# FurkanOM/tf-ssd

Measured on AMD Instinct MI355X. Metric: images/sec SSD300 (MobileNetV2) fwd+NMS, higher is better.
Workload: dtype f32

## Files before the change

include/ssd_hip.h:

```cpp
#ifndef SSD_HIP_H
#define SSD_HIP_H

#include <stddef.h>
#include <stdint.h>

#ifdef __cplusplus
extern "C" {
#endif

#define SSD_OK 0
#define SSD_E_INVALID (-1)
#define SSD_E_HIP (-2)
#define SSD_E_UNSUPPORTED (-3)
#define SSD_E_STATE (-4)

const char* ssd_version(void);
const char* ssd_last_error(void);
int ssd_init(int device);
void* ssd_stream_create(int high_priority);
void* ssd_stream_create_masked(const unsigned* cu_mask, int words);
int ssd_stream_destroy(void* stream);

int ssd_priors_count(const int* fmaps, const int* n_ars, int levels);
int ssd_priors(const int* fmaps, const float* const* ars, const int* n_ars, int levels,
// ... 364 lines not shown
    int B, H, W, Cin;
    int Cout, kh, kw;
    int stride, dilation;
    int pad_t, pad_l, pad_b, pad_r;
    int act;
    int has_residual;
} ssd_conv_desc;

int ssd_same_pads(int in, int k, int stride, int dilation, int* before, int* after);
int ssd_conv_out_size(int in, int k, int stride, int dilation, int pad_before, int pad_after);

size_t ssd_conv_packed_weight_floats(int kh, int kw, int Cin, int Cout);
int ssd_conv_pack_weights(const float* hwio_dev, int kh, int kw, int Cin, int Cout,
                          float* packed_dev, void* stream);

int ssd_conv2d(const ssd_conv_desc* d, const float* in_dev, const float* packed_w_dev,
               const float* scale_dev, const float* shift_dev, const float* residual_dev,
               float* out_dev, long out_batch_stride, long out_pixel_stride, void* stream);

int ssd_conv_num_configs(void);
const char* ssd_conv_config_name(int config);
int ssd_conv2d_ex(const ssd_conv_desc* d, const float* in_dev, const float* packed_w_dev,
                  const float* scale_dev, const float* shift_dev, const float* residual_dev,
                  float* out_dev, long out_batch_stride, long out_pixel_stride, int config,
                  int split_k, float* splitk_ws_dev, void* stream);

int ssd_split_planes(const float* x_dev, long n, int channels, int planes, void* planes_dev, long plane_stride, void* stream);
int ssd_join_planes(const void* planes_dev, long n, int channels, int planes, long plane_stride, float* x_dev, void* stream);
int ssd_conv2d_planes(const ssd_conv_desc* d, const void* in_planes_dev, int planes, long in_plane_stride,
                      const float* packed_w_dev, const float* scale_dev, const float* shift_dev,
                      const float* residual_dev, float* out_dev, long out_batch_stride, long out_pixel_stride,
                      void* out_planes_dev, long out_plane_stride, int config, int split_k,
                      float* splitk_ws_dev, void* stream);

size_t ssd_conv_f16x2_weight_bytes(int kh, int kw, int Cin, int Cout);
int ssd_conv_pack_weights_f16x2(const float* packed_w_dev, int kh, int kw, int Cin, int Cout, void* w_planes_dev,
                                int* k_out, void* stream);
int ssd_conv2d_planes_f16x2(const ssd_conv_desc* d, const void* in_planes_dev, long in_plane_stride,
                            const float* packed_w_dev, const void* w_planes_dev, int w_exp, const float* scale_dev,
                            const float* shift_dev, const float* residual_dev, float* out_dev,
                            long out_batch_stride, long out_pixel_stride, void* out_planes_dev,
                            long out_plane_stride, int config, int split_k, float* splitk_ws_dev, void* stream);

size_t ssd_conv_wino_weight_floats(int Cin, int Cout);
int ssd_conv_wino_pack_weights(const float* hwio_dev, int Cin, int Cout, float* wino_w_dev, void* stream);
int ssd_conv_wino_num_configs(void);
int ssd_conv2d_wino(const ssd_conv_desc* d, const float* in_dev, const float* wino_w_dev,
                    const float* scale_dev, const float* shift_dev, float* out_dev,
                    long out_batch_stride, long out_pixel_stride, int wino_config, int split_k,
                    float* splitk_ws_dev, void* stream);

int ssd_dwconv3x3(const float* in_dev, int B, int H, int W, int C, int stride,
                  int pad_t, int pad_l, int pad_b, int pad_r,
                  const float* w_dev, const float* scale_dev, const float* shift_dev,
                  int act, float* out_dev, void* stream);

int ssd_maxpool2d(const float* in_dev, int B, int H, int W, int C, int k, int stride,
                  int pad_t, int pad_l, int pad_b, int pad_r, float* out_dev, void* stream);

int ssd_l2norm(const float* in_dev, long pixels, int C, const float* gamma_dev,
               float* out_dev, void* stream);

int ssd_softmax(const float* in_dev, long rows, int L, float* out_dev, void* stream);

typedef struct ssd_net ssd_net;

enum ssd_backbone { SSD_MOBILENET_V2 = 0, SSD_VGG16 = 1 };

ssd_net* ssd_net_create(int backbone, int img_size, int levels, const int* n_ars,
                        int total_labels);
void ssd_net_destroy(ssd_net* net);

int ssd_net_num_params(const ssd_net* net);
const char* ssd_net_param_name(const ssd_net* net, int i);
int ssd_net_param_rank(const ssd_net* net, int i);
const int* ssd_net_param_shape(const ssd_net* net, int i);
int ssd_net_set_param(ssd_net* net, const char* name, const float* host_data, size_t count);
int ssd_net_get_param(const ssd_net* net, const char* name, float* host_out, size_t count);
int ssd_net_finalize(ssd_net* net, int max_batch);
long ssd_net_get_tuning(const ssd_net* net, char* buf, size_t cap);
int ssd_net_set_tuning(ssd_net* net, const char* text);
int ssd_net_tuning_stats(const ssd_net* net, int* from_table, int* timed);
int ssd_net_memory_bytes(const ssd_net* net, size_t out[4]);
const char* ssd_build_id(void);
int ssd_net_num_priors(const ssd_net* net);
int ssd_net_feature_map_size(const ssd_net* net, int level);

int ssd_net_forward(ssd_net* net, const float* image_dev, int B, float* deltas_out_dev,
                    float* probs_out_dev, void* stream);

int ssd_net_predict(ssd_net* net, const float* image_dev, int B, const float* priors_dev,
                    const float* var, int max_total, float iou_thr, float score_thr,
                    float* boxes_dev, float* labels_dev, float* scores_dev, int* valid_dev,
                    void* stream);
int ssd_net_predict_cfg(ssd_net* net, const float* image_dev, int B, const float* priors_dev, const float* var,
                        const ssd_nms_config* cfg, float* boxes_dev, float* labels_dev, float* scores_dev,
                        int* valid_dev, void* stream);

long ssd_net_fetch_activation(ssd_net* net, const char* layer, float* host_out, size_t cap);
long ssd_net_fetch_planes(ssd_net* net, const char* layer, float* host_out, size_t cap, int* planes_out);

int ssd_net_num_layers(const ssd_net* net);
const char* ssd_net_layer_name(const ssd_net* net, int i);
const char* ssd_net_layer_kind(const ssd_net* net, int i);
const char* ssd_net_layer_config(const ssd_net* net, int i);
double ssd_net_layer_flops(const ssd_net* net, int i, int B);
double ssd_net_layer_bytes(const ssd_net* net, int i, int B);
double ssd_net_layer_executed_flops(const ssd_net* net, int i, int B);
int ssd_net_set_option(ssd_net* net, const char* name, int value);
int ssd_net_set_timing(ssd_net* net, int enabled);
int ssd_net_read_timing(ssd_net* net, float* ms_sum_out, int* forwards_out);
int ssd_net_profile_layers(ssd_net* net, const float* image_dev, int B, int reps,
                           float* ms_out, void* stream);

int ssd_net_train_begin(ssd_net* net, int batch);
size_t ssd_net_trainable_floats(const ssd_net* net);
long ssd_net_trainable_offset(const ssd_net* net, const char* name);
int ssd_net_train_forward_backward(ssd_net* net, const float* image_dev, int B,
                                   const float* actual_deltas_dev, const float* actual_labels_dev,
                                   float neg_pos_ratio, float loc_loss_alpha, float* grads_flat_dev,
                                   float* loc_loss_dev, float* conf_loss_dev, void* stream);
int ssd_net_train_forward_backward_cfg(ssd_net* net, const float* image_dev, int B,
                                       const float* actual_deltas_dev, const float* actual_labels_dev,
                                       const ssd_loss_config* loss, float* grads_flat_dev,
                                       float* loc_loss_dev, float* conf_loss_dev, void* stream);
int ssd_net_train_set_buckets(ssd_net* net, int n, const long* lo);
int ssd_net_train_wait_bucket(ssd_net* net, int k, void* stream);
int ssd_net_adam_step(ssd_net* net, const float* grads_flat_dev, float lr, float beta1, float beta2,
                      float eps, float grad_scale, void* stream);
long ssd_net_train_steps(const ssd_net* net);
#define SSD_OPT_ADAM 0
#define SSD_OPT_SGD 1
typedef struct ssd_optimizer {
    int kind;
    float beta1, beta2, eps;
    float momentum;
    int nesterov;
    float clipnorm, clipvalue, global_clipnorm;
} ssd_optimizer;
int ssd_net_optimizer_step(ssd_net* net, const float* grads_flat_dev, const ssd_optimizer* opt, float lr,
                           float grad_scale, void* stream);
int ssd_net_optimizer_reset(ssd_net* net);
long ssd_net_optimizer_get_state(ssd_net* net, const char* slot, float* host_out, size_t cap);
int ssd_net_optimizer_set_state(ssd_net* net, const char* slot, const float* host_in, size_t count);
int ssd_net_train_set_steps(ssd_net* net, long steps);
int ssd_net_train_matrix_flops(const ssd_net* net, double* out3);
int ssd_net_regularization_loss(ssd_net* net, float* host_out);
int ssd_net_set_trainable(ssd_net* net, const char* keras_layer, int trainable);
int ssd_net_get_trainable(const ssd_net* net, const char* keras_layer);
#define SSD_PLAN_WGRAD 1
#define SSD_PLAN_WGRAD2 2
#define SSD_PLAN_DGRAD 4
#define SSD_PLAN_RESGRAD 8
#define SSD_PLAN_BN_BATCH 16
#define SSD_PLAN_BN_PARAMS 32
#define SSD_PLAN_SKIP 64
int ssd_net_train_plan(const ssd_net* net, int layer, int* flags);
long ssd_net_train_fetch(ssd_net* net, const char* what, int B, float* host_out, size_t cap);

int ssd_conv_wgrad_num_configs(void);
size_t ssd_conv_wgrad_workspace_floats(const ssd_conv_desc* d, int N);
int ssd_conv2d_wgrad_ex(const ssd_conv_desc* d, const float* x_dev, const float* g_dev, int ldg, int N, int config,
                        float* dW_dev, float* workspace_dev, size_t workspace_floats, void* stream);
int ssd_dwconv3x3_backward(const float* x_dev, const float* g_dev, const float* w_dev, int B, int H, int W, int C, int stride,
                           int pad_t, int pad_l, int accumulate, float* dx_dev, float* dw_dev, float* workspace_dev,
                           size_t workspace_floats, void* stream);

#ifdef __cplusplus
}
#endif
#endif
```

tf-ssd_amd/csrc/ssd_bf16x3.h:

```cpp
#pragma once
#include <hip/hip_runtime.h>

namespace ssd {

typedef float b3_f32x4 __attribute__((ext_vector_type(4)));
typedef short bf16x8 __attribute__((ext_vector_type(8)));

struct B3 {
    bf16x8 h, m, l;
};

__device__ __forceinline__ void split1(float x, short& h, short& m, short& l) {
    const unsigned hb = __float_as_uint(x) & 0xffff0000u;
    const float r1 = x - __uint_as_float(hb);
    const unsigned mb = __float_as_uint(r1) & 0xffff0000u;
    const float r2 = r1 - __uint_as_float(mb);
    h = (short)(hb >> 16);
    m = (short)(mb >> 16);
    l = (short)(__float_as_uint(r2) >> 16);
}
__device__ __forceinline__ void split4(const b3_f32x4 v, uint2& h, uint2& m, uint2& l) {
    unsigned hb[4], mb[4], lb[4];
#pragma unroll
    for (int j = 0; j < 4; ++j) {
        hb[j] = __float_as_uint(v[j]) & 0xffff0000u;
        const float r1 = v[j] - __uint_as_float(hb[j]);
        mb[j] = __float_as_uint(r1) & 0xffff0000u;
        lb[j] = __float_as_uint(r1 - __uint_as_float(mb[j]));
    }
    h = make_uint2(__builtin_amdgcn_perm(hb[1], hb[0], 0x07060302u), __builtin_amdgcn_perm(hb[3], hb[2], 0x07060302u));
    m = make_uint2(__builtin_amdgcn_perm(mb[1], mb[0], 0x07060302u), __builtin_amdgcn_perm(mb[3], mb[2], 0x07060302u));
    l = make_uint2(__builtin_amdgcn_perm(lb[1], lb[0], 0x07060302u), __builtin_amdgcn_perm(lb[3], lb[2], 0x07060302u));
}
__device__ __forceinline__ B3 split3(const b3_f32x4 a, const b3_f32x4 b) {
    B3 r;
#pragma unroll
    for (int j = 0; j < 4; ++j) {
        short h, m, l;
        split1(a[j], h, m, l);
        r.h[j] = h; r.m[j] = m; r.l[j] = l;
        split1(b[j], h, m, l);
        r.h[4 + j] = h; r.m[4 + j] = m; r.l[4 + j] = l;
    }
    return r;
}
__device__ __forceinline__ b3_f32x4 mma6(const B3& w, const B3& x, b3_f32x4 acc) {
    acc = __builtin_amdgcn_mfma_f32_16x16x32_bf16(w.m, x.m, acc, 0, 0, 0);
    acc = __builtin_amdgcn_mfma_f32_16x16x32_bf16(w.h, x.l, acc, 0, 0, 0);
    acc = __builtin_amdgcn_mfma_f32_16x16x32_bf16(w.l, x.h, acc, 0, 0, 0);
    acc = __builtin_amdgcn_mfma_f32_16x16x32_bf16(w.h, x.m, acc, 0, 0, 0);
    acc = __builtin_amdgcn_mfma_f32_16x16x32_bf16(w.m, x.h, acc, 0, 0, 0);
    acc = __builtin_amdgcn_mfma_f32_16x16x32_bf16(w.h, x.h, acc, 0, 0, 0);
    return acc;
}

typedef __bf16 bf16x2_t __attribute__((ext_vector_type(2)));
typedef float b3_f32x2 __attribute__((ext_vector_type(2)));

__device__ __forceinline__ unsigned rne2(float a, float b) {
    const bf16x2_t r = __builtin_convertvector(b3_f32x2{a, b}, bf16x2_t);
    return __builtin_bit_cast(unsigned, r);
}
__device__ __forceinline__ short rne1(float a) { return (short)(rne2(a, 0.f) & 0xffffu); }
__device__ __forceinline__ uint2 rne4(const b3_f32x4 v) { return make_uint2(rne2(v[0], v[1]), rne2(v[2], v[3])); }

typedef _Float16 f16x2_t __attribute__((ext_vector_type(2)));
typedef _Float16 f16x8 __attribute__((ext_vector_type(8)));
constexpr float kF16x2ActScale = 256.f;

__device__ __forceinline__ void split_h2(const float a, const float b, unsigned& h, unsigned& l) {
    const f16x2_t hh = __builtin_convertvector(b3_f32x2{a, b}, f16x2_t);
    const b3_f32x2 back = __builtin_convertvector(hh, b3_f32x2);
    const f16x2_t ll = __builtin_convertvector(b3_f32x2{a - back[0], b - back[1]}, f16x2_t);
    h = __builtin_bit_cast(unsigned, hh);
    l = __builtin_bit_cast(unsigned, ll);
}
__device__ __forceinline__ void split4_h(const b3_f32x4 v, uint2& h, uint2& l) {
    split_h2(v[0] * kF16x2ActScale, v[1] * kF16x2ActScale, h.x, l.x);
    split_h2(v[2] * kF16x2ActScale, v[3] * kF16x2ActScale, h.y, l.y);
}
__device__ __forceinline__ float join_h(const short h, const short l) {
    const float fh = (float)__builtin_bit_cast(_Float16, h), fl = (float)__builtin_bit_cast(_Float16, l);
    return (fh + fl) * (1.f / kF16x2ActScale);
}

template <int NP>
struct BP {
    bf16x8 p[NP];
};
template <int NP>
__device__ __forceinline__ BP<NP> splitN(const b3_f32x4 a, const b3_f32x4 b) {
    BP<NP> r;
    if constexpr (NP == 3) {
        const B3 s = split3(a, b);
        r.p[0] = s.h; r.p[1] = s.m; r.p[2] = s.l;
    } else {
        const uint4 u = make_uint4(rne2(a[0], a[1]), rne2(a[2], a[3]), rne2(b[0], b[1]), rne2(b[2], b[3]));
        r.p[0] = __builtin_bit_cast(bf16x8, u);
    }
    return r;
}
template <int NP>
__device__ __forceinline__ b3_f32x4 mmaN(const BP<NP>& w, const BP<NP>& x, b3_f32x4 acc) {
    if constexpr (NP == 2) {
        const f16x8 wh = __builtin_bit_cast(f16x8, w.p[0]), wl = __builtin_bit_cast(f16x8, w.p[1]);
        const f16x8 xh = __builtin_bit_cast(f16x8, x.p[0]), xl = __builtin_bit_cast(f16x8, x.p[1]);
        acc = __builtin_amdgcn_mfma_f32_16x16x32_f16(wl, xh, acc, 0, 0, 0);
        acc = __builtin_amdgcn_mfma_f32_16x16x32_f16(wh, xl, acc, 0, 0, 0);
        return __builtin_amdgcn_mfma_f32_16x16x32_f16(wh, xh, acc, 0, 0, 0);
    }
    if constexpr (NP == 3) {
        acc = __builtin_amdgcn_mfma_f32_16x16x32_bf16(w.p[1], x.p[1], acc, 0, 0, 0);
        acc = __builtin_amdgcn_mfma_f32_16x16x32_bf16(w.p[0], x.p[2], acc, 0, 0, 0);
        acc = __builtin_amdgcn_mfma_f32_16x16x32_bf16(w.p[2], x.p[0], acc, 0, 0, 0);
        acc = __builtin_amdgcn_mfma_f32_16x16x32_bf16(w.p[0], x.p[1], acc, 0, 0, 0);
        acc = __builtin_amdgcn_mfma_f32_16x16x32_bf16(w.p[1], x.p[0], acc, 0, 0, 0);
    }
    return __builtin_amdgcn_mfma_f32_16x16x32_bf16(w.p[0], x.p[0], acc, 0, 0, 0);
}
__device__ __forceinline__ void pack_planes(float x, int bf16_mode, short& h, short& m, short& l) {
    if (bf16_mode) { h = rne1(x); m = 0; l = 0; }
    else split1(x, h, m, l);
}

__device__ __host__ __forceinline__ long plane_elem(const long pix, const int c, const long P) {
    return (((long)(c >> 5) * P + pix) << 5) + (c & 31);
}
__device__ __forceinline__ void store_planes4(short* __restrict__ op, const long plane, const int np, const long pix, const int c,
                                              const long P, const b3_f32x4 v) {
    const long e = plane_elem(pix, c, P);
    if (np == 1) {
        *reinterpret_cast<uint2*>(op + e) = rne4(v);
    } else if (np == 2) {
        uint2 h, l;
        split4_h(v, h, l);
        *reinterpret_cast<uint2*>(op + e) = h;
        *reinterpret_cast<uint2*>(op + plane + e) = l;
    } else {
        uint2 h, m, l;
        split4(v, h, m, l);
        *reinterpret_cast<uint2*>(op + e) = h;
        *reinterpret_cast<uint2*>(op + plane + e) = m;
        *reinterpret_cast<uint2*>(op + 2 * plane + e) = l;
    }
}
__device__ __forceinline__ void store_planes4_lin(short* __restrict__ op, const long plane, const int np, const long e, const int C,
                                                  const long P, const b3_f32x4 v) {
    const long pix = e / C;
    store_planes4(op, plane, np, pix, (int)(e - pix * C), P, v);
}

}
```

tf-ssd_amd/csrc/ssd_conv.h:

```cpp
#pragma once
#include <cmath>
#include <cstring>

#include "common.h"

namespace ssd {

struct ConvParams {
    const float* in;
    const float* w;
    const short* w3;
    const float* scale;
    const float* shift;
    const float* residual;
    float* out;
    int B, H, W, Cin, Ho, Wo, Cout;
    int kh, kw, stride, dil, pad_t, pad_l;
    int K, Kpad, Npad;
    long M;
    long out_batch_stride, out_pixel_stride;
    int n_split;
    float* out2;
    long out2_batch_stride, out2_pixel_stride;
    int vec_store2;
    int act;
    int vec_store;
    int split_k;
    float* partial;
    const float* wino_w;
    int bf16;
    const short* xp;
    long xp_plane;
    int xp_np;
    short* op;
    long op_plane;
    int op_np;
    const short* wh;
    float acc_scale;
};
inline int conv_vec_store(const ConvParams& p) {
    return (((uintptr_t)p.out & 15) == 0) && (p.out_pixel_stride % 4 == 0) && (p.out_batch_stride % 4 == 0);
}

struct FusedBlockParams {
    const float* x;
    float* y;
    const float* we;
    const float *es, *eh;
    const float* wd;
    const float *ds, *dh;
    const float* wp;
    const float *ps, *ph;
    int residual;
    int B, H, W, Cin, Ce, Cout, Ho, Wo, stride, pad_t, pad_l;
    int kpad_e, kpad_p, npad_p;
    int tiles_y, tiles_x;
    int bf16;
    int groups;
    const short* we3;
    const short* wp3;
    int bands;
    float* slabs;
    unsigned* tickets;
    float* e_out;
    short* y_planes;
    long y_plane;
    short* e_planes;
    long e_plane;
    int planes_np;
    int e_planes_np;
    int planes_only;
    int form2;
};
struct StemParams {
    const float* x;
    float* y;
    const float* w1;
    const float *s1, *h1;
    const float* wd;
    const float *sd, *hd;
    const float* wp;
    const float *sp, *hp;
    int B, H, W, H1, W1, pad_t, pad_l, kpad1, kpadp;
    int tiles_y, tiles_x;
    int bf16;
};
struct DwProjParams {
    const float* e;
    const float* wd;
    const float* dh;
    const float* wp;
    const float* ph;
    const float* res;
    float* y;
    int B, H, W, Ce, Cout, Ho, Wo, stride, pad_t, pad_l;
    int kpad_p, npad_p;
    int tiles_y, tiles_x;
    int bf16;
};
bool dwproj_supported(const DwProjParams& p);
int launch_dwproj(DwProjParams p, hipStream_t st);
bool stem_supported(const StemParams& p);
int launch_stem(StemParams p, hipStream_t st);
bool image_block2_supported(const FusedBlockParams& p);
int launch_image_block2(FusedBlockParams p, hipStream_t st);
bool fused_block_supported(const FusedBlockParams& p);
int launch_fused_block(FusedBlockParams p, hipStream_t st);
bool band3_block_supported(const FusedBlockParams& p);
size_t band3_we_shorts(int Ce);
size_t band3_wp_shorts(int npad_p, int Ce);
int launch_band3_pack(const float* we, int Ce, int Cin, int kpad_e, short* we3, const float* wp, int npad_p, int kpad_p,
                      short* wp3, hipStream_t st);
int launch_band3_block(FusedBlockParams p, hipStream_t st);
bool band_block_supported(const FusedBlockParams& p);
int launch_band_block(FusedBlockParams p, hipStream_t st);
bool image_block_supported(const FusedBlockParams& p);
bool image_block_split_fits(FusedBlockParams p);
int image_block_groups(const FusedBlockParams& p, int B);
size_t image_block_slab_floats(const FusedBlockParams& p, int B);
int launch_image_block(FusedBlockParams p, hipStream_t st);

inline int round_up(int v, int a) { return (v + a - 1) / a * a; }
inline int conv_kpad(int K) { return round_up(K, 32); }
inline int conv_npad(int Cout) { return round_up(Cout, 16); }

enum ConvFamilyId { CF_NONE = -1, CF_MFMA, CF_WINO, CF_SKINNY, CF_MFMA3, CF_BF16, CF_DMA3, CF_DMAB, CF_DMAH, CF_DIRECT };
enum : unsigned {
    CONV_READS_FP32 = 0, CONV_READS_PLANES = 1, CONV_READS_F16X2 = 2, CONV_READS_MASK = 3,
    CONV_NET_FP32 = 4, CONV_NET_BF16 = 8,
    CONV_WRITES_PLANES = 16,
    CONV_SPLITK_REDUCE = 32,
};
struct ConvFamily {
    ConvFamilyId id;
    int (*count)();
    const char* (*name)(int i);
    bool (*valid)(int i, const ConvParams& p);
    long (*grid_blocks)(int i, const ConvParams& p);
    int (*k_tiles)(int i, const ConvParams& p);
    int (*launch)(const ConvParams& p, int i, hipStream_t st);
    unsigned traits;
};
extern const ConvFamily kConvMfma, kConvDirect;
extern const ConvFamily kConvWino;
extern const ConvFamily kConvSkinny;
extern const ConvFamily kConvMfma3, kConvBf16;
extern const ConvFamily kConvDma3, kConvDmab, kConvDmah;

int conv_num_configs();
const char* conv_config_name(int cfg);
ConvFamilyId conv_config_family(int cfg);
bool conv_config_valid(int cfg, const ConvParams& p);
bool conv_config_allowed(int cfg, int precision);
int conv_config_reads(int cfg);
bool conv_config_is_dma(int cfg);
bool conv_config_is_dmah(int cfg);
int conv_dmah_twin(int cfg);
bool conv_config_writes_planes(int cfg, const ConvParams& p);
int conv_pick_config(const ConvParams& p);
long conv_grid_blocks(int cfg, const ConvParams& p);
int conv_k_tiles(int cfg, const ConvParams& p);
int conv_launch(const ConvParams& p, int cfg, hipStream_t st);

int fill_conv_params(const ssd_conv_desc* d, ConvParams* p);
int launch_splitk_reduce(const ConvParams& p, hipStream_t st);
inline bool conv_is_gemm1x1(const ConvParams& p) {
    return p.kh == 1 && p.kw == 1 && p.stride == 1 && p.pad_t == 0 && p.pad_l == 0 && p.Ho == p.H && p.Wo == p.W;
}

bool wino_applicable(const ConvParams& p);
size_t wino_weight_floats(int Cin, int Cout);
int launch_wino_pack(const float* hwio, int Cin, int Cout, int Npad, int row_off, float* U, hipStream_t st);
void mfma3_tile(int i, int* BM, int* BN);
int dmah_tile_index(int j);
int launch_absmax_bits(const float* packed, int K, int Cout, unsigned* absmax_bits_dev, hipStream_t st);
int launch_pack_f16x2(const float* packed, int K, int Cout, int k, short* planes, hipStream_t st);
inline int conv_f16x2_weight_exp(unsigned absmax_bits) {
    float wmax;
    std::memcpy(&wmax, &absmax_bits, sizeof(float));
    if (!(wmax > 0.f)) return 0;
    int e = 0;
    (void)std::frexp(wmax, &e);
    return 14 - e;
}
inline size_t conv_f16x2_plane_shorts(int K, int Cout) { return (size_t)2 * conv_kpad(K) * conv_npad(Cout); }
int launch_split_planes(const float* x, long n, int C, int np, short* planes, long plane, hipStream_t st);
int launch_join_planes(const short* planes, long n, int C, int np, long plane, float* x, hipStream_t st);

int launch_dwconv3x3(const float* in, int B, int H, int W, int C, int stride, int pad_t, int pad_l,
                     int Ho, int Wo, const float* w, const float* scale, const float* shift, int act,
                     float* out, hipStream_t st);
int launch_maxpool(const float* in, int B, int H, int W, int C, int k, int stride, int pad_t, int pad_l,
                   int Ho, int Wo, float* out, hipStream_t st, short* planes = nullptr, long plane = 0, int np = 0);
int launch_l2norm(const float* in, long pixels, int C, const float* gamma, float* out, hipStream_t st,
                  short* planes = nullptr, long plane = 0, int np = 0);
int launch_softmax(const float* in, long rows, int L, float* out, hipStream_t st);
bool decode_nms_fused_ok(int L);
int decode_nms_fused(const float* deltas, const float* logits, const float* priors, const float* var, int B, int N, int L,
                     int max_per_class, int max_total, float iou_thr, float score_thr, float* boxes, float* labels,
                     float* scores, int* valid, void* ws, size_t ws_bytes, int ws_batch, hipStream_t st);
int decode_nms_fused_cfg(const float* deltas, const float* logits, const float* priors, const float* var, int B, int N, int L,
                         const ssd_nms_config* cfg, float* boxes, float* labels, float* scores, int* valid, void* ws,
                         size_t ws_bytes, int ws_batch, hipStream_t st);
int launch_pack_weights(const float* hwio, int K, int Cout, int Kpad, int Npad, float* packed, hipStream_t st);
inline size_t conv_packed_floats(int K, int Cout) {
    const size_t n = (size_t)conv_kpad(K) * conv_npad(Cout);
    return n + 2 * n;
}
inline const short* conv_split_planes(const float* packed, int K, int Cout) {
    return reinterpret_cast<const short*>(packed + (size_t)conv_kpad(K) * conv_npad(Cout));
}
int launch_pack_split(float* packed, int K, int Cout, hipStream_t st, bool row_major = false);
int launch_scale_rows(const float* in, const float* scale, int rows, int nvalid, int cols, float* out, hipStream_t st);
int launch_scale_cols(const float* in, const float* scale, int rows, int cols, float* out, hipStream_t st);
int launch_fold_bn(const float* gamma, const float* beta, const float* mean, const float* var, float eps,
                   int C, float* scale, float* shift, hipStream_t st);

}
```

tf-ssd_amd/csrc/ssd_convdma.hip:

```cpp
#include "ssd_block_common.h"
#include "ssd_conv_mfma.h"

namespace ssd {

template <int MT, int NT, int WM, int WN, int NP, bool GEMM1X1, int KSH = 1>
__device__ __forceinline__ void conv_dma_body(const ConvParams& p, char* __restrict__ dsm) {
    constexpr int KS = NP == 1 ? 2 : NP == 2 ? KSH : 1;
    constexpr int WPL = NP == 1 ? 3 : 0;
    constexpr int BM = 16 * MT * WM, BN = 16 * NT * WN, NW = WM * WN;
    constexpr int RBX = BM / 16, RBW = BN / 16;
    constexpr int RPX = (RBX + NW - 1) / NW, RPW = (RBW + NW - 1) / NW;
    constexpr int XBYTES = KS * NP * BM * 64, STAGE = KS * NP * (BM + BN) * 64;

    const int tid = threadIdx.x, lane = tid & 63;
    const int wave = __builtin_amdgcn_readfirstlane(tid >> 6);
    const int wm = wave / WN, wn = wave % WN;
    const int nb_n = (p.Cout + BN - 1) / BN;
    const int mblk = blockIdx.x / nb_n, nblk = blockIdx.x - mblk * nb_n;
    const long m0 = (long)mblk * BM;
    const int n0 = nblk * BN;
    const int HoWo = p.Ho * p.Wo;
    const int ntaps = p.kh * p.kw;

    const int r16 = lane >> 2;
// ... 199 lines not shown
    const char* name1;
    const char* nameh;
    const char* nameh2;
    int BM, BN, threads;
    convd_kernel_t gemm3, general3, gemm1, general1, gemmh, generalh, gemmh2, generalh2;
};
template <int MT, int NT, int WM, int WN, bool GEMM1X1>
constexpr convd_kernel_t dmah_ks2_kernel() {
    if constexpr (16 * MT * WM + 16 * NT * WN <= 320) return conv_dma_kernel<MT, NT, WM, WN, 2, GEMM1X1, 2>;
    else return nullptr;
}
#define DCFG(MT, NT, WM, WN)                                                                                  \
    {"dma3_" #MT "x" #NT "_" #WM "x" #WN, "dmab_" #MT "x" #NT "_" #WM "x" #WN, "dmah_" #MT "x" #NT "_" #WM "x" #WN,          \
     "dmah_" #MT "x" #NT "_" #WM "x" #WN "_ks2", 16 * MT * WM, 16 * NT * WN, 64 * WM * WN,                       \
     conv_dma_kernel<MT, NT, WM, WN, 3, true>, conv_dma_kernel<MT, NT, WM, WN, 3, false>,                       \
     conv_dma_kernel<MT, NT, WM, WN, 1, true>, conv_dma_kernel<MT, NT, WM, WN, 1, false>,                       \
     conv_dma_kernel<MT, NT, WM, WN, 2, true>, conv_dma_kernel<MT, NT, WM, WN, 2, false>,                       \
     dmah_ks2_kernel<MT, NT, WM, WN, true>(), dmah_ks2_kernel<MT, NT, WM, WN, false>()}
const ConvDCfg kCfgD[] = {
    DCFG(4, 4, 4, 2),
    DCFG(2, 4, 4, 2),
    DCFG(4, 4, 2, 4),
    DCFG(4, 2, 4, 2),
    DCFG(2, 7, 8, 1),
    DCFG(4, 5, 4, 2),
    DCFG(4, 4, 2, 2),
    DCFG(2, 7, 4, 1),
    DCFG(2, 5, 2, 2),
    DCFG(2, 4, 6, 2),
    DCFG(3, 4, 4, 3),
    DCFG(2, 4, 8, 2),
    DCFG(2, 2, 2, 2),
    DCFG(2, 5, 6, 2),
};
constexpr int kNumCfgD = sizeof(kCfgD) / sizeof(kCfgD[0]);
struct DmahList {
    int n = 0, tile[2 * kNumCfgD], ks[2 * kNumCfgD];
    DmahList() {
        for (int i = 0; i < kNumCfgD; ++i) { tile[n] = i; ks[n++] = 1; }
        for (int i = 0; i < kNumCfgD; ++i)
            if (kCfgD[i].gemmh2) { tile[n] = i; ks[n++] = 2; }
    }
};
const DmahList& dmah_list() {
    static const DmahList l;
    return l;
}

__global__ __launch_bounds__(256) void split_planes_kernel(const float* __restrict__ x, const long n4, const int C, const int np,
                                                           short* __restrict__ planes, const long plane) {
    const long P = n4 * 4 / C;
    for (long e = (long)blockIdx.x * 256 + threadIdx.x; e < n4; e += (long)gridDim.x * 256)
        store_planes4_lin(planes, plane, np, e * 4, C, P, *reinterpret_cast<const f32x4*>(x + e * 4));
}

__global__ __launch_bounds__(256) void join_planes_kernel(const short* __restrict__ planes, const long n, const int C, const int np,
                                                          const long plane, float* __restrict__ x) {
    const long P = n / C;
    for (long e = (long)blockIdx.x * 256 + threadIdx.x; e < n; e += (long)gridDim.x * 256) {
        const long pix = e / C;
        const long s = plane_elem(pix, (int)(e - pix * C), P);
        if (np == 2) {
            x[e] = join_h(planes[s], planes[plane + s]);
            continue;
        }
        float v = __uint_as_float((unsigned)(unsigned short)planes[s] << 16);
        if (np == 3) {
            v += __uint_as_float((unsigned)(unsigned short)planes[plane + s] << 16);
            v += __uint_as_float((unsigned)(unsigned short)planes[2 * plane + s] << 16);
        }
        x[e] = v;
    }
}

__global__ __launch_bounds__(256) void absmax_bits_kernel(const float* __restrict__ w, const long total, unsigned* __restrict__ out) {
    unsigned m = 0;
    for (long e = (long)blockIdx.x * 256 + threadIdx.x; e < total; e += (long)gridDim.x * 256) m = max(m, __float_as_uint(w[e]) & 0x7fffffffu);
    atomicMax(out, m);
}
__global__ __launch_bounds__(256) void pack_f16x2_kernel(const float* __restrict__ w, const long total, const int Kpad, const int Npad,
                                                         const float scale, short* __restrict__ out) {
    for (long e = (long)blockIdx.x * 256 + threadIdx.x; e < total; e += (long)gridDim.x * 256) {
        const long n = e / Kpad;
        const long d = plane_elem(n, (int)(e - n * Kpad), Npad);
        unsigned h, l;
        split_h2(w[e] * scale, 0.f, h, l);
        out[d] = (short)(h & 0xffffu);
        out[total + d] = (short)(l & 0xffffu);
    }
}

int dma_num_configs() { return kNumCfgD; }
const char* dma3_config_name(int i) { return kCfgD[i].name3; }
const char* dmab_config_name(int i) { return kCfgD[i].name1; }
bool dma_config_valid(int i, int np, const ConvParams& p) {
    const short* wpl = np == 2 ? p.wh : p.w3;
    if (!p.xp || !wpl || p.xp_np != np) return false;
    if (((uintptr_t)p.xp & 15) || ((uintptr_t)wpl & 15) || (p.xp_plane & 7)) return false;
    if (p.M > 0x7fffffffL - 1024) return false;
    if (4 * (long)p.Npad * p.Kpad * 2 > 0x7fffffffL) return false;
    if ((long)p.B * p.H * p.W * p.Cin * 2 > 0x7fffffffL) return false;
    if (conv_is_gemm1x1(p)) return p.Cin % 32 == 0;
    if (p.kh * p.kw > 32) return false;
    if (((long)kCfgD[i].BM / (p.Ho * p.Wo) + 3) * p.H * p.W * 64 > 0x3fffffffL) return false;
    return p.Cin % (np == 1 ? 64 : 32) == 0;
}
bool dma3_config_valid(int i, const ConvParams& p) { return dma_config_valid(i, 3, p); }
bool dmab_config_valid(int i, const ConvParams& p) { return dma_config_valid(i, 1, p); }
long dma_grid_blocks(int i, const ConvParams& p) {
    return ((p.M + kCfgD[i].BM - 1) / kCfgD[i].BM) * ((p.Cout + kCfgD[i].BN - 1) / kCfgD[i].BN);
}
int dma3_k_tiles(int, const ConvParams& p) { return (p.K + 31) / 32; }
int dmab_k_tiles(int, const ConvParams& p) { return (p.K + 31) / 32 / 2; }

int dma_launch(const ConvParams& p, int i, convd_kernel_t gemm, convd_kernel_t general, int stage_planes, hipStream_t st) {
    const long blocks = dma_grid_blocks(i, p);
    SSD_UNSUPPORTED_IF(blocks > 0x7fffffffL, "conv2d: grid too large");
    const ConvDCfg& g = kCfgD[i];
    const convd_kernel_t fn = conv_is_gemm1x1(p) ? gemm : general;
    const int lds = 2 * stage_planes * (g.BM + g.BN) * 64;
    if (lds > 64 * 1024) SSD_HIP(hipFuncSetAttribute(reinterpret_cast<const void*>(fn), hipFuncAttributeMaxDynamicSharedMemorySize, lds));
    dim3 grid((unsigned)blocks, p.split_k > 1 ? p.split_k : 1);
    hipLaunchKernelGGL(fn, grid, dim3(g.threads), lds, st, p);
    SSD_LAUNCH_CHECK();
    return SSD_OK;
}
int dma3_launch(const ConvParams& p, int i, hipStream_t st) { return dma_launch(p, i, kCfgD[i].gemm3, kCfgD[i].general3, 3, st); }
int dmab_launch(const ConvParams& p, int i, hipStream_t st) { return dma_launch(p, i, kCfgD[i].gemm1, kCfgD[i].general1, 2, st); }

int dmah_num_configs() { return dmah_list().n; }
const char* dmah_config_name(int j) {
    const DmahList& l = dmah_list();
    return l.ks[j] == 2 ? kCfgD[l.tile[j]].nameh2 : kCfgD[l.tile[j]].nameh;
}
bool dmah_config_valid(int j, const ConvParams& p) {
    if (!(p.acc_scale > 0.f)) return false;
    return dma_config_valid(dmah_list().tile[j], 2, p);
}
long dmah_grid_blocks(int j, const ConvParams& p) { return dma_grid_blocks(dmah_list().tile[j], p); }
int dmah_k_tiles(int j, const ConvParams& p) {
    const int ks = dmah_list().ks[j];
    if (conv_is_gemm1x1(p)) return ((p.K + 31) / 32 + ks - 1) / ks;
    return p.kh * p.kw * ((p.Cin / 32 + ks - 1) / ks);
}
int dmah_launch(const ConvParams& p, int j, hipStream_t st) {
    const ConvDCfg& g = kCfgD[dmah_list().tile[j]];
    if (dmah_list().ks[j] == 2) return dma_launch(p, dmah_list().tile[j], g.gemmh2, g.generalh2, 4, st);
    return dma_launch(p, dmah_list().tile[j], g.gemmh, g.generalh, 2, st);
}

}

#ifndef __HIP_DEVICE_COMPILE__
const ConvFamily kConvDma3 = {CF_DMA3, dma_num_configs, dma3_config_name, dma3_config_valid, dma_grid_blocks, dma3_k_tiles, dma3_launch,
                              CONV_READS_PLANES | CONV_NET_FP32 | CONV_WRITES_PLANES | CONV_SPLITK_REDUCE};
const ConvFamily kConvDmab = {CF_DMAB, dma_num_configs, dmab_config_name, dmab_config_valid, dma_grid_blocks, dmab_k_tiles, dmab_launch,
                              CONV_READS_PLANES | CONV_NET_BF16 | CONV_WRITES_PLANES | CONV_SPLITK_REDUCE};
const ConvFamily kConvDmah = {CF_DMAH, dmah_num_configs, dmah_config_name, dmah_config_valid, dmah_grid_blocks, dmah_k_tiles, dmah_launch,
                              CONV_READS_F16X2 | CONV_NET_FP32 | CONV_WRITES_PLANES | CONV_SPLITK_REDUCE};
#endif
int dmah_tile_index(int j) { return dmah_list().tile[j]; }

int launch_absmax_bits(const float* packed, int K, int Cout, unsigned* absmax_bits_dev, hipStream_t st) {
    const long total = (long)conv_kpad(K) * conv_npad(Cout);
    if (total == 0) return SSD_OK;
    const int blocks = (int)((total + 255) / 256 < 1024 ? (total + 255) / 256 : 1024);
    hipLaunchKernelGGL(absmax_bits_kernel, dim3(blocks), dim3(256), 0, st, packed, total, absmax_bits_dev);
    SSD_LAUNCH_CHECK();
    return SSD_OK;
}
int launch_pack_f16x2(const float* packed, int K, int Cout, int k, short* planes, hipStream_t st) {
    const long total = (long)conv_kpad(K) * conv_npad(Cout);
    if (total == 0) return SSD_OK;
    const int blocks = (int)((total + 255) / 256 < 8192 ? (total + 255) / 256 : 8192);
    hipLaunchKernelGGL(pack_f16x2_kernel, dim3(blocks), dim3(256), 0, st, packed, total, conv_kpad(K), conv_npad(Cout), ldexpf(1.f, k), planes);
    SSD_LAUNCH_CHECK();
    return SSD_OK;
}

int launch_split_planes(const float* x, long n, int C, int np, short* planes, long plane, hipStream_t st) {
    SSD_CHECK_ARG(n % 4 == 0 && np >= 1 && np <= 3, "split_planes: element count %ld must be a multiple of 4, planes 1, 2 or 3", n);
    SSD_CHECK_ARG(C > 0 && C % 32 == 0 && n % C == 0, "split_planes: %d channels (slice-major planes need a multiple of 32 that divides the %ld elements)", C, n);
    SSD_UNSUPPORTED_IF((((uintptr_t)x) & 15) || (((uintptr_t)planes) & 7) || (plane & 3),
                       "split_planes: needs a 16-byte aligned source and 8-byte aligned planes (16-byte loads, 8-byte stores)");
    if (n == 0) return SSD_OK;
    const long n4 = n / 4;
    const int blocks = (int)((n4 + 255) / 256 < 16384 ? (n4 + 255) / 256 : 16384);
    hipLaunchKernelGGL(split_planes_kernel, dim3(blocks), dim3(256), 0, st, x, n4, C, np, planes, plane);
    SSD_LAUNCH_CHECK();
    return SSD_OK;
}

int launch_join_planes(const short* planes, long n, int C, int np, long plane, float* x, hipStream_t st) {
    if (n == 0) return SSD_OK;
    SSD_CHECK_ARG(C > 0 && n % C == 0, "join_planes: %d channels do not divide the %ld elements", C, n);
    const int blocks = (int)((n + 255) / 256 < 16384 ? (n + 255) / 256 : 16384);
    hipLaunchKernelGGL(join_planes_kernel, dim3(blocks), dim3(256), 0, st, planes, n, C, np, plane, x);
    SSD_LAUNCH_CHECK();
    return SSD_OK;
}

}
```

tf-ssd_amd/csrc/ssd_imgblock.hip:

```cpp

#include "ssd_bf16x3.h"
#include "ssd_block_common.h"
#include "ssd_conv.h"

namespace ssd {

namespace {

constexpr int kIC = 16;
constexpr int kILD = 24;
constexpr int kIThreads = 512;

__device__ __forceinline__ void gstore16_sc1(float* ptr, f32x4 v) {
    asm volatile("global_store_dwordx4 %0, %1, off sc1\n\ts_nop 1" ::"v"(ptr), "v"(v) : "memory");
}

template <int CIN, int NT, int T, int S = 1>
__global__ __launch_bounds__(kIThreads) void mbv2_image_block_kernel(const FusedBlockParams p) {
    constexpr int TO = S == 1 ? T : 1;
    constexpr int KC = CIN / 16;
    constexpr int LDW = CIN + 8;
    constexpr int NCH = T == 1 ? 2 : 1;
    constexpr int WE_U = kIC * CIN / 4, WE_R = (WE_U + kIThreads - 1) / kIThreads;
    constexpr int WP_U = NT * 16 * kIC / 4, WP_R = (WP_U + kIThreads - 1) / kIThreads;
// ... 575 lines not shown
    ICFG(64, 4, 3),
    ICFG(64, 6, 3),
    ICFG(96, 6, 3),
    ICFG(160, 10, 1),
    ICFG(160, 20, 1),
    ICFG2(96, 10, 3),
};

size_t image_lds_bytes(const ImageCfg& c, const FusedBlockParams& p, int G) {
    const int P = p.W + 1, npt = (p.H * P + 15) / 16, NE = npt * 16 + 2 * P + 2;
    if (p.bf16) {
        const int np = p.bf16 == 3 ? 3 : 1, ks = c.cin / 32;
        const size_t w = (size_t)(2 * np * 16 * (ks * 32 + 16) + np * c.nt * 16 * 32) * sizeof(short);
        return ((size_t)2 * NE * kILD + (size_t)11 * (p.Ce / G) + 4) * sizeof(float) + w;
    }
    const size_t fl = (size_t)2 * NE * kILD + (size_t)2 * kIC * (c.cin + 8) + (size_t)2 * c.nt * 16 * kILD +
                      (size_t)11 * (p.Ce / G) + 4;
    return fl * sizeof(float);
}

const ImageCfg* pick_image(const FusedBlockParams& p) {
    if (p.Ce % kIC != 0 || p.Cout % 16 != 0 || p.kpad_e % 4 != 0 || p.kpad_p % 4 != 0) return nullptr;
    if (p.stride == 1 && (p.H != p.Ho || p.W != p.Wo)) return nullptr;
    if (p.stride == 2 && (p.residual || p.Ho != (p.H + 1) / 2 || p.Wo != (p.W + 1) / 2 || p.pad_t > 1 || p.pad_l > 1 ||
                          (p.Ho * (p.Wo + 1) + 15) / 16 > 8))
        return nullptr;
    if (p.stride != 1 && p.stride != 2) return nullptr;
    if (p.residual && p.Cin != p.Cout) return nullptr;
    const int npt = (p.H * (p.W + 1) + 15) / 16;
    FusedBlockParams q = p;
    if (q.bf16 == 3) q.bf16 = 0;
    for (const auto& c : kImage)
        if (c.cin == p.Cin && c.nt * 16 == p.Cout && c.stride == p.stride && npt <= 8 * c.t && npt > 8 * (c.t == 3 ? 1 : 0) &&
            image_lds_bytes(c, q, 1) <= 160 * 1024)
            return &c;
    return nullptr;
}

}

bool image_block_supported(const FusedBlockParams& p) { return pick_image(p) != nullptr; }
bool image_block_split_fits(FusedBlockParams p) {
    const ImageCfg* c = pick_image(p);
    p.bf16 = 3;
    return c && p.we3 && p.wp3 && image_lds_bytes(*c, p, p.groups < 1 ? 1 : p.groups) <= 160 * 1024;
}

int image_block_groups(const FusedBlockParams& p, int B) {
    static int num_cu = 0;
    if (!num_cu) {
        int dev = 0;
        (void)hipGetDevice(&dev);
        if (hipDeviceGetAttribute(&num_cu, hipDeviceAttributeMultiprocessorCount, dev) != hipSuccess || num_cu <= 0)
            num_cu = 256;
    }
    const int units = p.Ce / kIC;
    int best = 1;
    for (int g = 1; g <= 12 && g <= units; ++g) {
        if (units % g) continue;
        best = g;
        if ((long)B * g * 8 >= (long)num_cu * 7) break;
    }
    return best;
}

size_t image_block_slab_floats(const FusedBlockParams& p, int B) {
    const int G = image_block_groups(p, B);
    return G > 1 ? (size_t)G * B * p.Ho * p.Wo * p.Cout : 0;
}

int launch_image_block(FusedBlockParams p, hipStream_t st) {
    const ImageCfg* c = pick_image(p);
    if (!c) {
        set_error("image block: unsupported shape Cin=%d Ce=%d Cout=%d %dx%d stride=%d", p.Cin, p.Ce, p.Cout, p.H, p.W, p.stride);
        return SSD_E_UNSUPPORTED;
    }
    if (p.B == 0) return SSD_OK;
    if (p.groups < 1) p.groups = 1;
    SSD_CHECK_ARG(!(p.planes_only & 1) || p.y_planes, "image block: plane-only y without planes");
    SSD_CHECK_ARG(!(p.planes_only & 2) || (p.e_out && p.e_planes), "image block: plane-only expanded map without planes");
    SSD_CHECK_ARG(!p.planes_only || !p.tickets, "image block: plane-only outputs combine by the second launch only");
    SSD_CHECK_ARG((p.Ce / kIC) % p.groups == 0, "image block: %d groups do not divide Ce/16 = %d", p.groups, p.Ce / kIC);
    SSD_CHECK_ARG(p.groups == 1 || p.slabs, "image block: %d groups need the slab workspace", p.groups);
    if (p.bf16 == 3 && image_lds_bytes(*c, p, p.groups) > 160 * 1024) p.bf16 = 0;
    const size_t lds = image_lds_bytes(*c, p, p.groups);
    SSD_UNSUPPORTED_IF(lds > 160 * 1024, "image block: needs %zu B of LDS", lds);
    SSD_CHECK_ARG(!p.bf16 || (p.we3 && p.wp3), "image block: the bf16 form needs the weights' bf16 planes");
    SSD_CHECK_ARG(!p.bf16 || !p.tickets, "image block: the bf16 form combines by the second launch only");
    const image_kernel_t fn = p.bf16 == 3 ? c->fn3 : p.bf16 ? c->fn16 : c->fn;
    const bool second = p.form2 && p.bf16 && !p.tickets && image_block2_supported(p);
    if (second) {
        const int rc = launch_image_block2(p, st);
        if (rc) return rc;
    }
    if (lds > 64 * 1024 && !second)
        SSD_HIP(hipFuncSetAttribute((const void*)fn, hipFuncAttributeMaxDynamicSharedMemorySize, (int)lds));
    if (!second) {
        hipLaunchKernelGGL(fn, dim3((unsigned)((long)p.B * p.groups)), dim3(kIThreads), lds, st, p);
        SSD_LAUNCH_CHECK();
    }
    if (p.groups > 1 && !p.tickets) {
        const long nvec = (long)p.B * p.Ho * p.Wo * p.Cout / 4;
        const int blocks = (int)((nvec + 255) / 256 < 4096 ? (nvec + 255) / 256 : 4096);
        hipLaunchKernelGGL(image_combine_kernel, dim3(blocks), dim3(256), 0, st, p.slabs, p.ph, p.residual ? p.x : nullptr, p.y,
                           nvec, nvec, p.groups, p.Cout / 4, p.y_planes, p.y_plane, p.planes_np, p.planes_only & 1);
        SSD_LAUNCH_CHECK();
    }
    return SSD_OK;
}

}
```

tf-ssd_amd/csrc/ssd_imgblock2.hip:

```cpp

#include "ssd_bf16x3.h"
#include "ssd_block_common.h"
#include "ssd_conv.h"

namespace ssd {

namespace {

constexpr int kC = 16;

template <int CIN, int NT, int NW, int T, int H, int W, int NP, int LOOP, int S = 1>
__device__ __forceinline__ void image16v2_body(const FusedBlockParams& p, float* __restrict__ sm2) {
    static_assert(CIN % 32 == 0, "whole 32-channel k-steps");
    constexpr int NTH = NW * 64;
    constexpr int P = W + 1, Q = H * P;
    static_assert(NW * 16 * T >= Q, "the waves' pixel slots cover the padded map");
    constexpr int NPIX = NW * 16 * T;
    constexpr int NE = NPIX + 2 * P + 2;
    constexpr int ROW = S == 2 ? 20 : (T & 1) ? 24 : 20;
    static_assert(((S == 2 ? 2 : T) * ROW) % 16 == 8, "neighbouring lanes must sit 8 (mod 16) words apart");
    constexpr int TO = S == 1 ? T : 1;
    constexpr int Ho = S == 1 ? H : (H + 1) / 2, Wo = S == 1 ? W : (W + 1) / 2, Po = Wo + 1;
    static_assert(S == 1 || NW * 16 >= Ho * Po, "stride 2: one output pixel per lane covers the output map");
    constexpr int WPL = NP == 1 ? 3 : 0;
    constexpr int KS = CIN / 32;
    constexpr int EBUF = NE * ROW;
    constexpr int PCH = 11 * kC;
    constexpr int NBE = NP * KS, NBP = NP * NT;

    const int tid = threadIdx.x, lane = tid & 63, wave = tid >> 6, l15 = lane & 15, g4 = lane >> 4;
    const int wave_s = __builtin_amdgcn_readfirstlane(wave);
    const int G = p.groups, B = p.B;
    const int grp = blockIdx.x / B, img = blockIdx.x - grp * B;
    const int pairs_total = p.Ce / (2 * kC), pq = pairs_total / G, pr = pairs_total - pq * G;
    const int npairs = pq + (grp < pr ? 1 : 0), pair0 = grp * pq + min(grp, pr);
    const int cbeg = pair0 * 2 * kC, nchunk = 2 * npairs, CeG = nchunk * kC;
    const int CeGmax = (pq + (pr ? 1 : 0)) * 2 * kC;

    float* Es = sm2;
    float* Ps = Es + 2 * EBUF;
    short* Wes = reinterpret_cast<short*>(Ps + 11 * CeGmax);
    short* Wps = Wes + 2 * NBE * 512;
    const long plane_e = (long)p.Ce * p.kpad_e, plane_p = (long)p.npad_p * p.kpad_p;

    const __amdgpu_buffer_rsrc_t rs_e = __builtin_amdgcn_make_buffer_rsrc(const_cast<short*>(p.we3 + WPL * plane_e), 0, (int)(NP * plane_e * 2), 0x00020000);
    const __amdgpu_buffer_rsrc_t rs_p = __builtin_amdgcn_make_buffer_rsrc(const_cast<short*>(p.wp3 + WPL * plane_p), 0, (int)(NP * plane_p * 2), 0x00020000);
    const int dr = lane >> 2, dq8 = ((lane & 3) ^ ((lane >> 3) & 3)) * 8;
    const int voff_e = ((((dr >> 2) * 8 + (dr & 3)) * p.kpad_e) + dq8) * 2;
    const int voff_p = (dr * p.kpad_p + dq8) * 2;
    auto dma_we = [&](const int j, const int stage) {
        const int ch0 = cbeg + (j >> 1) * 32 + (j & 1) * 4;
        for (int b = wave_s; b < NBE; b += NW) {
            const int pl = b / KS, ks = b - pl * KS;
            __builtin_amdgcn_raw_ptr_buffer_load_lds(rs_e, (lds_dst_t)(Wes + (stage * NBE + b) * 512), 16, voff_e,
                                                     (int)((pl * plane_e + (long)ch0 * p.kpad_e + ks * 32) * 2), 0, 0);
        }
    };
    auto dma_wp = [&](const int pair) {
        for (int b = wave_s; b < NBP; b += NW) {
            const int pl = b / NT, nb = b - pl * NT;
            __builtin_amdgcn_raw_ptr_buffer_load_lds(rs_p, (lds_dst_t)(Wps + b * 512), 16, voff_p,
                                                     (int)((pl * plane_p + (long)nb * 16 * p.kpad_p + cbeg + pair * 32) * 2), 0, 0);
        }
    };
    auto dma_wait = [&]() { asm volatile("s_waitcnt vmcnt(0)" ::: "memory"); };
    dma_we(0, 0);
    dma_we(1, 1);
    dma_wp(0);

    for (int u = tid; u < 2 * (2 * P + 2) * (ROW / 4); u += NTH) {
        const int buf = u / ((2 * P + 2) * (ROW / 4)), v = u - buf * ((2 * P + 2) * (ROW / 4));
        const int row = v / (ROW / 4), c4 = (v - row * (ROW / 4)) * 4;
        const int e = row < P + 1 ? row : NPIX + row;
        *reinterpret_cast<f32x4*>(Es + buf * EBUF + e * ROW + c4) = f32x4{0.f, 0.f, 0.f, 0.f};
    }
    const int q0 = (wave * 16 + l15) * T;
    BP<NP> xs[T][KS];
    bool real[T];
    int opix[T];
#pragma unroll
    for (int t = 0; t < T; ++t) {
        const int q = q0 + t;
        const int r = q / P, c = q - r * P;
        real[t] = q < Q && c < W;
        opix[t] = real[t] ? r * W + c : 0;
        const float* xp = p.x + ((long)img * (H * W) + opix[t]) * CIN + g4 * 8;
#pragma unroll
        for (int ks = 0; ks < KS; ++ks) {
            const f32x4 lo = real[t] ? *reinterpret_cast<const f32x4*>(xp + ks * 32) : f32x4{0.f, 0.f, 0.f, 0.f};
            const f32x4 hi = real[t] ? *reinterpret_cast<const f32x4*>(xp + ks * 32 + 4) : f32x4{0.f, 0.f, 0.f, 0.f};
            xs[t][ks] = splitN<NP>(lo, hi);
        }
    }
    for (int u = tid; u < 11 * (CeG / 4); u += NTH) {
        const int row = u / (CeG / 4), c4 = (u - row * (CeG / 4)) * 4;
        const float* src = row == 0 ? p.eh : row == 10 ? p.dh : p.wd + (long)(row - 1) * p.Ce;
        const int w = c4 & 31, j = 2 * (c4 >> 5) + ((w >> 2) & 1), r = (w >> 3) * 4;
        *reinterpret_cast<f32x4*>(Ps + (j * 11 + row) * kC + r) = *reinterpret_cast<const f32x4*>(src + cbeg + c4);
    }
    dma_wait();
    __syncthreads();

    const float* e_rd = Es + (q0 + P + 1) * ROW + g4 * 4;
    float* e_wr = Es + (q0 + P + 1) * ROW + g4 * 4;
    const float* ps_l = Ps + g4 * 4;
    const int fslot = l15 * 32 + ((g4 ^ ((l15 >> 1) & 3)) * 8);
    const short* we_l = Wes + fslot;
    const short* wp_l = Wps + fslot;
    float relu_hi[T];
#pragma unroll
    for (int t = 0; t < T; ++t) relu_hi[t] = real[t] ? 6.0f : 0.0f;
    bool realo[TO];
    int opo[TO];
    if constexpr (S == 1) {
#pragma unroll
        for (int t = 0; t < T; ++t) { realo[t] = real[t]; opo[t] = opix[t]; }
    } else {
        const int qo = wave * 16 + l15, ro = qo / Po, co = qo - ro * Po;
        const bool in = qo < Ho * Po;
        realo[0] = in && co < Wo;
        opo[0] = realo[0] ? ro * Wo + co : 0;
        e_rd = Es + ((in ? (2 * ro - p.pad_t + 1) * P + (2 * co - p.pad_l + 1) : 0) + P + 1) * ROW + g4 * 4;
    }

    auto expand = [&](const int j, const int pb) {
        f32x4 ea[T];
        const f32x4 sh = *reinterpret_cast<const f32x4*>(ps_l + j * PCH);
#pragma unroll
        for (int t = 0; t < T; ++t) ea[t] = sh;
        const short* wl = we_l + pb * NBE * 512;
#pragma unroll
        for (int ks = 0; ks < KS; ++ks) {
            BP<NP> wea;
#pragma unroll
            for (int pl = 0; pl < NP; ++pl) wea.p[pl] = *reinterpret_cast<const bf16x8*>(wl + (pl * KS + ks) * 512);
#pragma unroll
            for (int t = 0; t < T; ++t) ea[t] = mmaN<NP>(wea, xs[t][ks], ea[t]);
        }
        float* ew = e_wr + pb * EBUF;
#pragma unroll
        for (int t = 0; t < T; ++t) {
            f32x4 v = ea[t];
#pragma unroll
            for (int e = 0; e < 4; ++e) v[e] = __builtin_amdgcn_fmed3f(v[e], 0.0f, relu_hi[t]);
            *reinterpret_cast<f32x4*>(ew + t * ROW) = v;
            if (S == 2 && p.e_out && real[t]) {
                const int ch = cbeg + (j >> 1) * 32 + g4 * 8 + (j & 1) * 4;
                if (!(p.planes_only & 2)) *reinterpret_cast<f32x4*>(p.e_out + ((long)img * (H * W) + opix[t]) * p.Ce + ch) = v;
                if (p.e_planes) store_planes4(p.e_planes, p.e_plane, p.e_planes_np, (long)img * (H * W) + opix[t], ch, (long)B * (H * W), v);
            }
        }
    };
    auto depthwise = [&](const int i, const int pb, f32x4 (&a)[TO]) {
        const float* pc = ps_l + i * PCH;
        const f32x4 dh = *reinterpret_cast<const f32x4*>(pc + 10 * kC);
#pragma unroll
        for (int t = 0; t < TO; ++t) a[t] = dh;
        const float* es = e_rd + pb * EBUF;
#pragma unroll
        for (int dy = -1; dy <= 1; ++dy) {
            f32x4 w[3], e[TO + 2];
#pragma unroll
            for (int dx = 0; dx < 3; ++dx) w[dx] = *reinterpret_cast<const f32x4*>(pc + (1 + (dy + 1) * 3 + dx) * kC);
#pragma unroll
            for (int j = 0; j < TO + 2; ++j)
                e[j] = *reinterpret_cast<const f32x4*>(es + (dy * P + j - 1) * ROW);
#pragma unroll
            for (int dx = 0; dx < 3; ++dx)
#pragma unroll
                for (int t = 0; t < TO; ++t) a[t] += e[t + dx] * w[dx];
        }
#pragma unroll
        for (int t = 0; t < TO; ++t)
#pragma unroll
            for (int e = 0; e < 4; ++e) a[t][e] = __builtin_amdgcn_fmed3f(a[t][e], 0.0f, 6.0f);
    };
    f32x4 acc[TO][NT];
#pragma unroll
    for (int t = 0; t < TO; ++t)
#pragma unroll
        for (int ni = 0; ni < NT; ++ni) acc[t][ni] = f32x4{0.f, 0.f, 0.f, 0.f};
    auto project = [&](const f32x4 (&a0)[TO], const f32x4 (&a1)[TO]) {
        BP<NP> d[TO];
#pragma unroll
        for (int t = 0; t < TO; ++t) d[t] = splitN<NP>(a0[t], a1[t]);
#pragma unroll
        for (int ni = 0; ni < NT; ++ni) {
            BP<NP> wa;
#pragma unroll
            for (int pl = 0; pl < NP; ++pl) wa.p[pl] = *reinterpret_cast<const bf16x8*>(wp_l + (pl * NT + ni) * 512);
#pragma unroll
            for (int t = 0; t < TO; ++t) acc[t][ni] = mmaN<NP>(wa, d[t], acc[t][ni]);
        }
    };

    expand(0, 0);

    if constexpr (LOOP == 0) {
        f32x4 dprev[TO];
        for (int c = 0; c < nchunk; ++c) {
            dma_wait();
            lds_barrier();
            const int pb = c & 1;
            if (c + 2 < nchunk) dma_we(c + 2, pb);
            if (!pb && c > 0) dma_wp(c >> 1);
            f32x4 a[TO];
            depthwise(c, pb, a);
            if (!pb) {
#pragma unroll
                for (int t = 0; t < TO; ++t) dprev[t] = a[t];
            } else {
                project(dprev, a);
            }
            if (c + 1 < nchunk) expand(c + 1, pb ^ 1);
        }
    } else {
        for (int i = 0; i < nchunk; i += 2) {
            f32x4 a0[TO], a1[TO];
            dma_wait();
            lds_barrier();
            if (i + 2 < nchunk) dma_we(i + 2, 0);
            if (i > 0) dma_wp(i >> 1);
            depthwise(i, 0, a0);
            expand(i + 1, 1);
            dma_wait();
            lds_barrier();
            if (i + 3 < nchunk) dma_we(i + 3, 1);
            depthwise(i + 1, 1, a1);
            project(a0, a1);
            if (i + 2 < nchunk) expand(i + 2, 0);
        }
    }

    const long img_off = (long)img * (Ho * Wo) * p.Cout;
    if (G == 1) {
#pragma unroll
        for (int t = 0; t < TO; ++t) {
            if (!realo[t]) continue;
            float* yp = p.y + img_off + (long)opo[t] * p.Cout + g4 * 4;
#pragma unroll
            for (int ni = 0; ni < NT; ++ni) {
                f32x4 v = acc[t][ni] + *reinterpret_cast<const f32x4*>(p.ph + ni * 16 + g4 * 4);
                if (S == 1 && p.residual)
                    v = v + *reinterpret_cast<const f32x4*>(p.x + img_off + (long)opo[t] * p.Cout + ni * 16 + g4 * 4);
                if (!(p.planes_only & 1)) *reinterpret_cast<f32x4*>(yp + ni * 16) = v;
                if (p.y_planes) store_planes4(p.y_planes, p.y_plane, p.planes_np, (long)img * (Ho * Wo) + opo[t], g4 * 4 + ni * 16, (long)B * (Ho * Wo), v);
            }
        }
        return;
    }
    const long slab_stride = (long)B * (Ho * Wo) * p.Cout;
    float* sp = p.slabs + (long)grp * slab_stride + img_off + g4 * 4;
#pragma unroll
    for (int t = 0; t < TO; ++t) {
        if (!realo[t]) continue;
#pragma unroll
        for (int ni = 0; ni < NT; ++ni) *reinterpret_cast<f32x4*>(sp + (long)opo[t] * p.Cout + ni * 16) = acc[t][ni];
    }
}

template <int CIN, int NT, int NW, int T, int H, int W, int NP, int LOOP, int S = 1>
__global__ __launch_bounds__(NW * 64) void mbv2_image16v2_kernel(const FusedBlockParams p) {
    extern __shared__ __attribute__((aligned(1024))) float sm2[];
    image16v2_body<CIN, NT, NW, T, H, W, NP, LOOP, S>(p, sm2);
}

typedef void (*image2_kernel_t)(const FusedBlockParams);
struct Image2Cfg {
    int cin, nt, nw, t, h, w, stride;
    image2_kernel_t fn1, fn3;
};
#define I2CFG(CIN, NT, NW, T, H, W, LOOP) {CIN, NT, NW, T, H, W, 1, mbv2_image16v2_kernel<CIN, NT, NW, T, H, W, 1, LOOP>, mbv2_image16v2_kernel<CIN, NT, NW, T, H, W, 3, LOOP>}
#define I2CFG2(CIN, NT, NW, T, H, W, LOOP) {CIN, NT, NW, T, H, W, 2, mbv2_image16v2_kernel<CIN, NT, NW, T, H, W, 1, LOOP, 2>, mbv2_image16v2_kernel<CIN, NT, NW, T, H, W, 3, LOOP, 2>}
const Image2Cfg kImage2[] = {
    I2CFG(64, 4, 8, 3, 19, 19, 1),
    I2CFG(64, 6, 8, 3, 19, 19, 1),
    I2CFG(96, 6, 8, 3, 19, 19, 0),
    I2CFG2(96, 10, 8, 3, 19, 19, 0),
    I2CFG(160, 10, 8, 1, 10, 10, 1),
    I2CFG(160, 20, 8, 1, 10, 10, 1),
};


size_t image2_lds_bytes(const Image2Cfg& c, const FusedBlockParams& p, int G) {
    const int P = c.w + 1, npix = c.nw * 16 * c.t, NE = npix + 2 * P + 2, row = c.stride == 2 ? 20 : (c.t & 1) ? 24 : 20;
    const int np = p.bf16 == 3 ? 3 : 1, ks = c.cin / 32;
    const size_t w = (size_t)(2 * np * ks + np * c.nt) * 1024;
    const int pairs = p.Ce / (2 * kC), cmax = ((pairs + G - 1) / G) * 2 * kC;
    return ((size_t)2 * NE * row + (size_t)11 * cmax) * sizeof(float) + w;
}

const Image2Cfg* pick_image2(const FusedBlockParams& p) {
    if (!p.bf16 || p.Ce % (2 * kC) != 0 || p.kpad_e % 32 != 0 || p.kpad_p % 32 != 0) return nullptr;
    if (p.stride == 1 && (p.e_out || p.H != p.Ho || p.W != p.Wo)) return nullptr;
    if (p.stride == 2 && (p.residual || p.Ho != (p.H + 1) / 2 || p.Wo != (p.W + 1) / 2 || p.pad_t < 0 || p.pad_t > 1 || p.pad_l < 0 || p.pad_l > 1)) return nullptr;
    if (p.stride != 1 && p.stride != 2) return nullptr;
    if (p.residual && p.Cin != p.Cout) return nullptr;
    for (const auto& c : kImage2)
        if (c.cin == p.Cin && c.nt * 16 == p.Cout && c.h == p.H && c.w == p.W && c.stride == p.stride && p.kpad_e == c.cin && p.npad_p >= c.nt * 16) return &c;
    return nullptr;
}

}

bool image_block2_supported(const FusedBlockParams& p) {
    const Image2Cfg* c = pick_image2(p);
    const int G = p.groups < 1 ? 1 : p.groups;
    return c && p.we3 && p.wp3 && G <= p.Ce / (2 * kC) && image2_lds_bytes(*c, p, G) <= 160 * 1024;
}

int launch_image_block2(FusedBlockParams p, hipStream_t st) {
    const Image2Cfg* c = pick_image2(p);
    if (!c) {
        set_error("image block (second form): unsupported shape Cin=%d Ce=%d Cout=%d %dx%d stride=%d", p.Cin, p.Ce, p.Cout, p.H, p.W, p.stride);
        return SSD_E_UNSUPPORTED;
    }
    if (p.B == 0) return SSD_OK;
    if (p.groups < 1) p.groups = 1;
    SSD_CHECK_ARG(p.groups <= p.Ce / (2 * kC), "image block (second form): %d groups of %d chunk pairs", p.groups, p.Ce / (2 * kC));
    SSD_CHECK_ARG(p.groups == 1 || p.slabs, "image block: %d groups need the slab workspace", p.groups);
    SSD_CHECK_ARG(p.we3 && p.wp3, "image block: the bf16 forms need the weights' bf16 planes");
    const size_t lds = image2_lds_bytes(*c, p, p.groups);
    SSD_UNSUPPORTED_IF(lds > 160 * 1024, "image block (second form): needs %zu B of LDS", lds);
    const image2_kernel_t fn = p.bf16 == 3 ? c->fn3 : c->fn1;
    if (lds > 64 * 1024)
        SSD_HIP(hipFuncSetAttribute((const void*)fn, hipFuncAttributeMaxDynamicSharedMemorySize, (int)lds));
    hipLaunchKernelGGL(fn, dim3((unsigned)((long)p.B * p.groups)), dim3(c->nw * 64), lds, st, p);
    SSD_LAUNCH_CHECK();
    return SSD_OK;
}

}
```

tf-ssd_amd/csrc/ssd_net.h:

```cpp
#pragma once
#include <map>
#include <set>
#include <string>
#include <vector>

#include "ssd_conv.h"

struct ssd_train_state;
void ssd_train_state_free(ssd_train_state*);

namespace ssd {

enum LayerKind { LK_CONV = 0, LK_DW, LK_POOL, LK_L2NORM, LK_SOFTMAX, LK_FUSED };
static const char* kKindName[] = {"conv", "dw", "pool", "l2norm", "softmax", "fused"};

enum Route { RT_OFF = 0, RT_LAYER, RT_STEM, RT_DWPROJ, RT_TILE, RT_BAND, RT_BAND3, RT_IMAGE, RT_IMAGE_SPLIT };

struct Param {
    std::string name;
    std::vector<int> shape;
    size_t count = 0;
    float* dev = nullptr;
    bool set = false;
    bool in_flat = false;
};

struct Tensor {
    std::string name;
    int H = 0, W = 0, C = 0;
    size_t per_image = 0;
    float* dev = nullptr;
    short* planes = nullptr;
    long plane_stride = 0;
    int planes_np = 0;
    int planes_cap = 0;
    bool planes_live = false;
    bool plane_only = false;
};

struct Layer {
    std::string name;
    LayerKind kind = LK_CONV;
    int in = -1, out = -1, res = -1;
    int H = 0, W = 0, Cin = 0, Ho = 0, Wo = 0, Cout = 0;
    int kh = 1, kw = 1, stride = 1, dil = 1, pt = 0, pl = 0, pb = 0, pr = 0, act = 0;
    int p_kernel = -1, p_bias = -1, p_bn = -1;
    int p_kernel2 = -1, p_bias2 = -1, Cout1 = 0;
    int p_gamma = -1;
    int head_kind = 0;
    long head_off = 0, head_bs = 0, head_ps = 0;
    long head2_off = 0, head2_bs = 0, head2_ps = 0;
    float* packed = nullptr;
    float* wino = nullptr;
    float* scale = nullptr;
    float* shift = nullptr;
    int cfg = -1;
    int split_k = 1;
    float* wh = nullptr;
    int wh_k = 0;
    int f_expand = -1, f_dw = -1, f_project = -1;
    int f_type = 0;
    int fused_by = -1;
    int e_out = -1;
    int img_choice = -1;
    int fused_by2 = -1;
    Route route = RT_OFF;
    float* splitk_part = nullptr;
    float *fz_we = nullptr, *fz_wd = nullptr, *fz_wp = nullptr;
    float *fz_we3 = nullptr, *fz_wp3 = nullptr;
    int side = 0;
    hipEvent_t ev_ready = nullptr;
};

inline void conv_route_head(ConvParams& p, const Layer& l, float* probs, float* deltas) {
    p.out = probs + l.head_off;
    p.out_pixel_stride = l.head_ps;
    p.out_batch_stride = l.head_bs;
    p.n_split = l.Cout1;
    p.out2 = deltas + l.head2_off;
    p.out2_pixel_stride = l.head2_ps;
    p.out2_batch_stride = l.head2_bs;
    p.vec_store2 = (p.out2_pixel_stride % 4 == 0) && (p.out2_batch_stride % 4 == 0);
}

struct ScopedDev {
    float* p = nullptr;
    ~ScopedDev() { if (p) (void)hipFree(p); }
};
struct ScopedEvent {
    hipEvent_t e = nullptr;
    ~ScopedEvent() { if (e) (void)hipEventDestroy(e); }
};

struct Step {
    int layer = -1;
    int sid = -1;
    int wait[2] = {-1, -1};
    bool after_main = false;
    bool publishes = false;
    bool join_first = false;
};

}

struct ssd_net {
    int backbone = 0, img_size = 300, levels = 6, L = 21;
    std::vector<int> n_ars;
    std::vector<ssd::Param> params;
    std::map<std::string, int> param_index;
    std::vector<ssd::Tensor> tensors;
    std::map<std::string, int> tensor_index;
    std::vector<ssd::Layer> layers;
    std::vector<int> fmap;
    std::vector<long> level_off;
    int num_priors = 0;
    bool finalized = false;
    bool fuse_blocks = true;
    bool fuse_softmax = true;
    bool fuse_dwproj = true;
    bool use_wino = true;
    int precision = 0;
    int fuse_band = 2;
    int fuse_image = 1;
    int lanes_hint = 1;
    bool tail_on_side = false;
    bool image_split = true;
    bool image_v2 = true;
    bool conv_dma = true;
    bool conv_f16x2 = true;
    bool plane_only = true;
    bool image_ticket = false;
    float* img_slabs = nullptr;
    unsigned* img_tickets = nullptr;
    int max_batch = 0;
    int last_batch = 0;
    std::vector<float*> owned;
    float* arena = nullptr;
    size_t arena_bytes = 0, plane_bytes = 0, slab_bytes = 0;
    size_t wplane_bytes = 0;
    float* splitk_ws = nullptr;
    size_t splitk_floats = 0;
    float* deltas = nullptr;
    float* probs = nullptr;
    void* nms_ws = nullptr;
    size_t nms_ws_bytes = 0;
    int nms_ws_batch = 0;
    int nms_ws_total = 0;
    int scratch_batch = 0;
    std::map<std::string, std::pair<std::string, int>> preset;
    int n_preset = 0;
    int n_autotuned = 0;
    bool launch_raced = false;
    bool use_graph = true;
    bool graphs_unsafe = false;
    bool use_graph_auto = true;
    struct GraphEntry {
        std::vector<const void*> key;
        hipGraphExec_t exec = nullptr;
        hipGraph_t graph = nullptr;
        const float* image = nullptr;
        int batch = 0;
    };
    std::vector<GraphEntry> graphs;
    hipStream_t gstream = nullptr;
    bool overlap_heads = true;
    static constexpr int kSides = 2;
    hipStream_t side[kSides] = {nullptr, nullptr};
    hipEvent_t ev_side_done[kSides] = {nullptr, nullptr};
    std::vector<ssd::Step> steps;
    float* splitk_layers = nullptr;
    bool timing = false;
    ssd_train_state* train = nullptr;
    std::set<std::string> frozen;
    unsigned trainable_rev = 0;
    std::vector<std::vector<hipEvent_t>> timing_events;

    ~ssd_net() {
        for (auto& p : params)
            if (p.dev && !p.in_flat) (void)hipFree(p.dev);
        if (train) ssd_train_state_free(train);
        for (float* p : owned)
            if (p) (void)hipFree(p);
        if (arena) (void)hipFree(arena);
        if (splitk_ws) (void)hipFree(splitk_ws);
        if (deltas) (void)hipFree(deltas);
        if (probs) (void)hipFree(probs);
        if (nms_ws) (void)hipFree(nms_ws);
        for (auto& v : timing_events)
            for (auto e : v) (void)hipEventDestroy(e);
        drop_graphs();
        if (gstream) (void)hipStreamDestroy(gstream);
        for (int k = 0; k < kSides; ++k) {
            if (side[k]) (void)hipStreamDestroy(side[k]);
            if (ev_side_done[k]) (void)hipEventDestroy(ev_side_done[k]);
        }
        for (auto& l : layers)
            if (l.ev_ready) (void)hipEventDestroy(l.ev_ready);
        if (splitk_layers) (void)hipFree(splitk_layers);
    }
    void drop_graphs() {
        steps.clear();
        for (auto& g : graphs) {
            if (g.exec) (void)hipGraphExecDestroy(g.exec);
            if (g.graph) (void)hipGraphDestroy(g.graph);
        }
        graphs.clear();
    }
};
```

tf-ssd_amd/csrc/ssd_net.hip:

```cpp
#include <algorithm>
#include <cstdlib>
#include <cstring>
#include <map>
#include <memory>
#include <string>
#include <vector>

#include "ssd_net.h"

using namespace ssd;

namespace ssd {

struct Builder {
    ssd_net& net;
    explicit Builder(ssd_net& n) : net(n) {}

    int add_param(const std::string& name, std::vector<int> shape) {
        Param p;
        p.name = name;
        p.shape = std::move(shape);
        p.count = 1;
        for (int d : p.shape) p.count *= (size_t)d;
        net.params.push_back(p);
// ... 262 lines not shown
    p.w3 = conv_split_planes(l.packed, l.kh * l.kw * l.Cin, l.Cout);
    p.bf16 = net.precision;
    if (l.wh) {
        p.wh = reinterpret_cast<const short*>(l.wh);
        p.acc_scale = ldexpf(1.f, -(8 + l.wh_k));
    }
    if (l.in >= 0 && net.tensors[l.in].planes) {
        const Tensor& ti = net.tensors[l.in];
        p.xp = ti.planes; p.xp_plane = ti.plane_stride; p.xp_np = ti.planes_np;
    }
    if (l.out >= 0 && l.head_kind == 0 && net.tensors[l.out].planes_live && (l.Cout & 3) == 0) {
        const Tensor& to = net.tensors[l.out];
        p.op = to.planes; p.op_plane = to.plane_stride; p.op_np = to.planes_np;
    }
    p.wino_w = l.wino;
    p.scale = l.scale;
    p.shift = l.shift;
    p.residual = res;
    p.B = B; p.H = l.H; p.W = l.W; p.Cin = l.Cin; p.Ho = l.Ho; p.Wo = l.Wo; p.Cout = l.Cout;
    p.kh = l.kh; p.kw = l.kw; p.stride = l.stride; p.dil = l.dil; p.pad_t = l.pt; p.pad_l = l.pl;
    p.K = l.kh * l.kw * l.Cin;
    p.Kpad = conv_kpad(p.K);
    p.Npad = conv_npad(l.Cout);
    p.M = (long)B * l.Ho * l.Wo;
    p.act = l.act;
    p.split_k = l.split_k;
    p.partial = l.splitk_part ? l.splitk_part : net.splitk_ws;
    if (l.head_kind == 0) {
        p.out = l.out >= 0 && net.tensors[l.out].plane_only && p.op ? nullptr : out;
        p.out_pixel_stride = l.Cout;
        p.out_batch_stride = (long)l.Ho * l.Wo * l.Cout;
    } else {
        conv_route_head(p, l, probs_out, deltas_out);
    }
    p.vec_store = conv_vec_store(p);
    return p;
}

static FusedBlockParams fused_shape(const ssd_net& net, const Layer& f, int B) {
    const Layer& le = net.layers[f.f_expand];
    const Layer& ld = net.layers[f.f_dw];
    const Layer& lp = net.layers[f.f_project];
    FusedBlockParams p{};
    p.x = net.tensors[f.in].dev;
    p.y = net.tensors[f.out].dev;
    p.we = f.fz_we; p.es = le.scale; p.eh = le.shift;
    p.wd = f.fz_wd; p.ds = ld.scale; p.dh = ld.shift;
    p.wp = f.fz_wp; p.ps = lp.scale; p.ph = lp.shift;
    p.residual = lp.res >= 0 ? 1 : 0;
    p.B = B; p.H = f.H; p.W = f.W; p.Cin = f.Cin; p.Ce = le.Cout; p.Cout = f.Cout;
    p.Ho = f.Ho; p.Wo = f.Wo; p.stride = f.stride; p.pad_t = f.pt; p.pad_l = f.pl;
    p.kpad_e = conv_kpad(le.Cin);
    p.kpad_p = conv_kpad(lp.Cin);
    p.npad_p = conv_npad(lp.Cout);
    p.e_out = f.e_out >= 0 ? net.tensors[f.e_out].dev : nullptr;
    if (f.out >= 0 && net.tensors[f.out].planes_live) {
        const Tensor& to = net.tensors[f.out];
        p.y_planes = to.planes; p.y_plane = to.plane_stride; p.planes_np = to.planes_np;
    }
    if (f.e_out >= 0 && net.tensors[f.e_out].planes_live) {
        const Tensor& te = net.tensors[f.e_out];
        p.e_planes = te.planes; p.e_plane = te.plane_stride; p.e_planes_np = te.planes_np;
    }
    if (f.route == RT_IMAGE || f.route == RT_IMAGE_SPLIT)
        p.planes_only = (p.y_planes && net.tensors[f.out].plane_only ? 1 : 0) | (p.e_planes && net.tensors[f.e_out].plane_only ? 2 : 0);
    p.we3 = reinterpret_cast<const short*>(f.fz_we3);
    p.wp3 = reinterpret_cast<const short*>(f.fz_wp3);
    p.bf16 = net.precision;
    p.form2 = net.image_v2 ? 1 : 0;
    return p;
}

static FusedBlockParams fused_params(const ssd_net& net, const Layer& f, int B) {
    FusedBlockParams p = fused_shape(net, f, B);
    if (f.route == RT_IMAGE || f.route == RT_IMAGE_SPLIT) {
        const Layer& le = net.layers[f.f_expand];
        const Layer& lp = net.layers[f.f_project];
        p.we3 = conv_split_planes(f.fz_we, le.Cin, le.Cout);
        p.wp3 = conv_split_planes(f.fz_wp, lp.Cin, lp.Cout);
        p.groups = net.img_slabs ? image_block_groups(p, B * net.lanes_hint) : 1;
        p.slabs = net.img_slabs;
        p.tickets = net.image_ticket && !p.bf16 ? net.img_tickets : nullptr;
        if (f.route == RT_IMAGE_SPLIT) { p.bf16 = 3; p.tickets = nullptr; }
    }
    return p;
}

static DwProjParams dwproj_params(const ssd_net& net, const Layer& f, int B) {
    const Layer& ld = net.layers[f.f_dw];
    const Layer& lp = net.layers[f.f_project];
    DwProjParams p{};
    p.e = net.tensors[f.in].dev;
    p.y = net.tensors[f.out].dev;
    p.wd = f.fz_wd; p.dh = ld.shift;
    p.wp = f.fz_wp; p.ph = lp.shift;
    p.res = lp.res >= 0 ? net.tensors[lp.res].dev : nullptr;
    p.B = B; p.H = f.H; p.W = f.W; p.Ce = ld.Cout; p.Cout = f.Cout;
    p.Ho = f.Ho; p.Wo = f.Wo; p.stride = f.stride; p.pad_t = f.pt; p.pad_l = f.pl;
    p.kpad_p = conv_kpad(lp.Cin);
    p.npad_p = conv_npad(lp.Cout);
    p.bf16 = net.precision;
    return p;
}

static StemParams stem_params(const ssd_net& net, const Layer& f, int B) {
    const Layer& l1 = net.layers[f.f_expand];
    const Layer& ld = net.layers[f.f_dw];
    const Layer& lp = net.layers[f.f_project];
    StemParams p{};
    p.x = net.tensors[f.in].dev;
    p.y = net.tensors[f.out].dev;
    p.w1 = l1.packed; p.s1 = l1.scale; p.h1 = l1.shift;
    p.wd = net.params[ld.p_kernel].dev; p.sd = ld.scale; p.hd = ld.shift;
    p.wp = lp.packed; p.sp = lp.scale; p.hp = lp.shift;
    p.B = B; p.H = f.H; p.W = f.W; p.H1 = f.Ho; p.W1 = f.Wo; p.pad_t = f.pt; p.pad_l = f.pl;
    p.kpad1 = conv_kpad(27);
    p.kpadp = conv_kpad(32);
    p.bf16 = net.precision;
    return p;
}

static int planes_pass(ssd_net& net, int tensor, int B, hipStream_t st) {
    Tensor& t = net.tensors[tensor];
    return launch_split_planes(t.dev, (long)B * (long)t.per_image, t.C, t.planes_np, t.planes, t.plane_stride, st);
}

static int run_layer_kernels(ssd_net& net, const Layer& l, int B, float* deltas_out, float* probs_out, hipStream_t st,
                             int cfg_override) {
    const float* in = l.in >= 0 ? net.tensors[l.in].dev : nullptr;
    float* out = l.out >= 0 ? net.tensors[l.out].dev : nullptr;
    switch (l.kind) {
        case LK_CONV: {
            const float* res = l.res >= 0 ? net.tensors[l.res].dev : nullptr;
            ConvParams p = layer_conv_params(net, l, B, in, out, res, deltas_out, probs_out);
            const int cfg = cfg_override >= 0 ? cfg_override : l.cfg;
            const int rc = conv_launch(p, cfg, st);
            if (!rc && p.op && !conv_config_writes_planes(cfg, p)) return planes_pass(net, l.out, B, st);
            return rc;
        }
        case LK_DW:
            return launch_dwconv3x3(in, B, l.H, l.W, l.Cin, l.stride, l.pt, l.pl, l.Ho, l.Wo,
                                    net.params[l.p_kernel].dev, l.scale, l.shift, l.act, out, st);
        case LK_POOL: {
            const Tensor& to = net.tensors[l.out];
            return launch_maxpool(in, B, l.H, l.W, l.Cin, l.kh, l.stride, l.pt, l.pl, l.Ho, l.Wo, to.plane_only ? nullptr : out, st,
                                  to.planes_live ? to.planes : nullptr, to.plane_stride, to.planes_np);
        }
        case LK_L2NORM: {
            const Tensor& to = net.tensors[l.out];
            return launch_l2norm(in, (long)B * l.H * l.W, l.Cin, net.params[l.p_gamma].dev, to.plane_only ? nullptr : out, st,
                                 to.planes_live ? to.planes : nullptr, to.plane_stride, to.planes_np);
        }
        case LK_SOFTMAX:
            return launch_softmax(probs_out, (long)B * net.num_priors, net.L, probs_out, st);
        case LK_FUSED:
            switch (l.route) {
                case RT_STEM: return launch_stem(stem_params(net, l, B), st);
                case RT_DWPROJ: return launch_dwproj(dwproj_params(net, l, B), st);
                case RT_TILE: return launch_fused_block(fused_params(net, l, B), st);
                case RT_BAND: return launch_band_block(fused_params(net, l, B), st);
                case RT_BAND3: return launch_band3_block(fused_params(net, l, B), st);
                case RT_IMAGE:
                case RT_IMAGE_SPLIT: return launch_image_block(fused_params(net, l, B), st);
                default: break;
            }
            set_error("run_layer: no fused kernel is routed to layer %s", l.name.c_str());
// ... 46 lines not shown
    if (!image_block_supported(p)) return RT_OFF;
    return f.img_choice == 2 && net.precision == 0 ? RT_IMAGE_SPLIT : RT_IMAGE;
}

static void resolve_routes(ssd_net& net) {
    for (Layer& l : net.layers) {
        const bool owned = (l.fused_by >= 0 && net.layers[l.fused_by].route != RT_OFF) ||
                           (l.fused_by2 >= 0 && net.layers[l.fused_by2].route != RT_OFF);
        l.route = l.kind == LK_FUSED ? fused_route(net, l) : owned ? RT_OFF : RT_LAYER;
    }
}
static bool layer_runs(const Layer& l) { return l.route != RT_OFF; }

template <typename F>
static std::vector<char> plane_only_candidates(const ssd_net& net, F reads_planes) {
    const int nt = (int)net.tensors.size();
    std::vector<char> ok(nt, 0), readers(nt, 0);
    if (!net.plane_only || net.image_ticket) return ok;
    for (int t = 1; t < nt; ++t) ok[t] = net.tensors[t].planes != nullptr;
    auto bar = [&](int t) { if (t >= 0) ok[t] = 0; };
    for (int i = 0; i < (int)net.layers.size(); ++i) {
        const Layer& l = net.layers[i];
        if (!layer_runs(l)) continue;
        if (l.kind == LK_CONV && l.in >= 0 && reads_planes(i)) readers[l.in] = 1;
        else bar(l.in);
        bar(l.res);
        if (l.kind == LK_FUSED && l.f_project >= 0) bar(net.layers[l.f_project].res);
        const bool image = l.kind == LK_FUSED && (l.route == RT_IMAGE || l.route == RT_IMAGE_SPLIT);
        bool writes = image || l.kind == LK_POOL || l.kind == LK_L2NORM;
        if (l.kind == LK_CONV)
            writes = l.head_kind == 0 && (l.Cout & 3) == 0 && l.cfg >= 0 && conv_config_writes_planes(l.cfg, ConvParams{});
        if (!writes) { bar(l.out); bar(l.e_out); }
    }
    for (int t = 0; t < nt; ++t) ok[t] = ok[t] && readers[t];
    return ok;
}

static bool tensor_relu6_bounded(const ssd_net& net, int t) {
    if (net.precision != 0 || t < 1) return false;
    bool any = false;
    for (const Layer& l : net.layers) {
        if (l.kind == LK_FUSED && l.e_out == t) {
            const Layer& le = net.layers[l.f_expand];
            if (le.act != SSD_ACT_RELU6 || le.res >= 0) return false;
            any = true;
            continue;
        }
        if (l.out != t) continue;
        if (l.kind != LK_CONV || l.act != SSD_ACT_RELU6 || l.res >= 0 || l.head_kind != 0) return false;
        any = true;
    }
    return any;
}

static int dev_alloc(ssd_net& net, size_t floats, float** out) {
    *out = nullptr;
    if (floats == 0) return SSD_OK;
    SSD_HIP(hipMalloc((void**)out, floats * sizeof(float)));
    net.owned.push_back(*out);
    return SSD_OK;
}

static int tune_image_blocks(ssd_net& net, int B, hipStream_t st) {
    ScopedEvent se0, se1;
    SSD_HIP(hipEventCreate(&se0.e));
    SSD_HIP(hipEventCreate(&se1.e));
    struct ModeGuard {
        ssd_net& n;
        int mode;
        ~ModeGuard() { n.fuse_image = mode; }
    } guard{net, net.fuse_image};
    net.fuse_image = 1;
    int rc = SSD_OK;
    for (size_t fi = 0; fi < net.layers.size() && !rc; ++fi) {
        Layer& f = net.layers[fi];
        if (f.kind != LK_FUSED || f.f_type != 0) continue;
        if (!image_kernel_takes(net, f)) { f.img_choice = 0; continue; }
        if (f.img_choice >= 0) continue;
        float ms[3] = {1e30f, 1e30f, 1e30f};
        const int nchoice = net.precision == 0 && net.image_split ? 3 : 2;
        for (int choice = 0; choice < nchoice && !rc; ++choice) {
            f.img_choice = choice;
            resolve_routes(net);
            if (choice == 2 && !image_block_split_fits(fused_params(net, f, B))) continue;
            for (int trial = 0; trial < 4 && !rc; ++trial) {
                (void)hipEventRecord(se0.e, st);
                for (int r = 0; r < 4 && !rc; ++r)
                    for (int j = (int)fi; j <= f.f_project && !rc; ++j)
                        if (layer_runs(net.layers[j])) rc = run_layer(net, net.layers[j], B, nullptr, nullptr, st);
                (void)hipEventRecord(se1.e, st);
                if (rc) break;
                SSD_HIP(hipEventSynchronize(se1.e));
                float t = 0.f;
                (void)hipEventElapsedTime(&t, se0.e, se1.e);
                if (trial && t < ms[choice]) ms[choice] = t;
            }
        }
        f.img_choice = ms[2] < ms[1] && ms[2] < ms[0] ? 2 : ms[1] < ms[0] ? 1 : 0;
    }
    return rc;
}

static int autotune(ssd_net& net, int B, hipStream_t st) {
    ScopedEvent se0, se1;
    SSD_HIP(hipEventCreate(&se0.e));
    SSD_HIP(hipEventCreate(&se1.e));
    hipEvent_t e0 = se0.e, e1 = se1.e;
    ScopedDev sd, spr;
    SSD_HIP(hipMalloc((void**)&sd.p, (size_t)B * net.num_priors * 4 * sizeof(float)));
    SSD_HIP(hipMalloc((void**)&spr.p, (size_t)B * net.num_priors * net.L * sizeof(float)));
    float *d = sd.p, *pr = spr.p;
    static const int kSplits[] = {1, 2, 3, 4, 5, 6, 7, 8, 10, 12, 14, 16, 20, 24, 32};
    constexpr int kNumSplits = sizeof(kSplits) / sizeof(kSplits[0]);
    size_t ws_floats = 0;
    for (auto& l : net.layers) {
        if (l.kind != LK_CONV) continue;
        const size_t mc = (size_t)B * l.Ho * l.Wo * l.Cout;
        if (mc <= (size_t)4 << 20) ws_floats = std::max(ws_floats, mc * 32);
    }
    if (ws_floats > net.splitk_floats) {
        if (net.splitk_ws) (void)hipFree(net.splitk_ws);
        net.splitk_ws = nullptr;
        SSD_HIP(hipMalloc((void**)&net.splitk_ws, ws_floats * sizeof(float)));
        net.splitk_floats = ws_floats;
    }
    int rc = SSD_OK;
    const bool dbg_sync = getenv("SSD_HIP_DEBUG_SYNC") != nullptr;
    const bool dbg_tune = getenv("SSD_HIP_DEBUG_TUNE") != nullptr;
    struct Best {
        float ms[3] = {1e30f, 1e30f, 1e30f}; int cfg[3] = {-1, -1, -1}; int split[3] = {1, 1, 1}; bool timed = false;
        float ms_k64 = 1e30f, ms_k32 = 1e30f;
    };
    std::vector<Best> bests(net.layers.size());
    constexpr int kReps = 4;
    for (size_t li = 0; li < net.layers.size(); ++li) {
        Layer& l = net.layers[li];
        Best& bb = bests[li];
        if (l.kind != LK_CONV) continue;
        if (l.cfg >= 0) continue;
        bb.timed = true;
        const float* in = net.tensors[l.in].dev;
        float* out = l.out >= 0 ? net.tensors[l.out].dev : nullptr;
        const float* res = l.res >= 0 ? net.tensors[l.res].dev : nullptr;
        for (int c = 0; c < conv_num_configs() && !rc; ++c) {
            const int fam = conv_config_reads(c);
            if (fam == CONV_READS_F16X2 && (!net.conv_f16x2 || !l.wh)) continue;
            for (int si = 0; si < kNumSplits && !rc; ++si) {
                const int split = kSplits[si];
                l.split_k = split;
                ConvParams p = layer_conv_params(net, l, B, in, out, res, d, pr);
                if (fam == CONV_READS_F16X2) p.xp_np = 2;
                if (!conv_config_valid(c, p) || !conv_config_allowed(c, net.precision)) break;
                const bool direct = conv_config_family(c) == CF_DIRECT;
                if (direct && (bb.cfg[0] >= 0 || bb.cfg[1] >= 0 || split > 1)) break;
                if (split > 1) {
                    const long blocks = conv_grid_blocks(c, p);
                    const int nkt = conv_k_tiles(c, p);
                    if (blocks > 384 || nkt < 4 * split) break;
                    if ((size_t)split * p.M * p.Cout > net.splitk_floats) break;
                }
                const int reps = kReps;
                if (dbg_sync) fprintf(stderr, "[ssd dbg] tune %s %s split %d\n", l.name.c_str(), conv_config_name(c), split);
                rc = conv_launch(p, c, st);
                if (rc) break;
                if (dbg_sync) SSD_HIP(hipStreamSynchronize(st));
                float ms = 1e30f;
                for (int trial = 0; trial < 3 && !rc; ++trial) {
// ... 305 lines not shown
            l.wh_k = conv_f16x2_weight_exp(bits);
            rc = dev_alloc(*net, (conv_f16x2_plane_shorts(K, l.Cout) + 1) / 2, &l.wh);
            if (!rc) rc = launch_pack_f16x2(l.packed, K, l.Cout, l.wh_k, reinterpret_cast<short*>(l.wh), st);
            if (rc) return rc;
        }
    }
    if (l.kh == 3 && l.kw == 3 && l.stride == 1 && l.dil == 1 && l.Cin % 16 == 0 && l.res < 0 && net->use_wino) {
        const int np = conv_npad(l.Cout);
        rc = dev_alloc(*net, wino_weight_floats(l.Cin, l.Cout), &l.wino);
        if (rc) return rc;
        SSD_HIP(hipMemsetAsync(l.wino, 0, wino_weight_floats(l.Cin, l.Cout) * sizeof(float), st));
        if (l.p_kernel2 < 0) {
            rc = launch_wino_pack(net->params[l.p_kernel].dev, l.Cin, l.Cout, np, 0, l.wino, st);
        } else {
            rc = launch_wino_pack(net->params[l.p_kernel].dev, l.Cin, l.Cout1, np, 0, l.wino, st);
            if (!rc) rc = launch_wino_pack(net->params[l.p_kernel2].dev, l.Cin, l.Cout - l.Cout1, np, l.Cout1, l.wino, st);
        }
    }
    return rc;
}

static int finalize_fold_bn(ssd_net* net, Layer& l, hipStream_t st) {
    if (l.p_bn >= 0) {
        int rc = dev_alloc(*net, l.Cout, &l.scale);
        if (!rc) rc = dev_alloc(*net, l.Cout, &l.shift);
        if (rc) return rc;
        return launch_fold_bn(net->params[l.p_bn].dev, net->params[l.p_bn + 1].dev, net->params[l.p_bn + 2].dev,
                              net->params[l.p_bn + 3].dev, 1e-3f, l.Cout, l.scale, l.shift, st);
    }
    if (l.p_bias2 >= 0) {
        const int rc = dev_alloc(*net, l.Cout, &l.shift);
        if (rc) return rc;
        SSD_HIP(hipMemcpyAsync(l.shift, net->params[l.p_bias].dev, (size_t)l.Cout1 * sizeof(float),
                               hipMemcpyDeviceToDevice, st));
        SSD_HIP(hipMemcpyAsync(l.shift + l.Cout1, net->params[l.p_bias2].dev,
                               (size_t)(l.Cout - l.Cout1) * sizeof(float), hipMemcpyDeviceToDevice, st));
    } else if (l.p_bias >= 0) {
        l.shift = net->params[l.p_bias].dev;
    }
    return SSD_OK;
}

static int finalize_fused_weights(ssd_net* net, hipStream_t st) {
    for (auto& f : net->layers) {
        if (f.kind == LK_FUSED && f.f_type == 2) {
            const Layer& ld = net->layers[f.f_dw];
            const Layer& lp = net->layers[f.f_project];
            const size_t nd = (size_t)9 * ld.Cout, np = (size_t)conv_kpad(lp.Cin) * conv_npad(lp.Cout);
            int rc = dev_alloc(*net, nd, &f.fz_wd);
            if (!rc) rc = dev_alloc(*net, np, &f.fz_wp);
            if (rc) return rc;
            rc = launch_scale_cols(net->params[ld.p_kernel].dev, ld.scale, 9, ld.Cout, f.fz_wd, st);
            if (!rc) rc = launch_scale_rows(lp.packed, lp.scale, conv_npad(lp.Cout), lp.Cout, conv_kpad(lp.Cin), f.fz_wp, st);
            if (rc) return rc;
            continue;
        }
        if (f.kind != LK_FUSED || f.f_type != 0) continue;
        const Layer& le = net->layers[f.f_expand];
        const Layer& ld = net->layers[f.f_dw];
        const Layer& lp = net->layers[f.f_project];
        const size_t nd = (size_t)9 * ld.Cout;
        int rc = dev_alloc(*net, conv_packed_floats(le.Cin, le.Cout), &f.fz_we);
        if (!rc) rc = dev_alloc(*net, nd, &f.fz_wd);
        if (!rc) rc = dev_alloc(*net, conv_packed_floats(lp.Cin, lp.Cout), &f.fz_wp);
        if (rc) return rc;
        rc = launch_scale_rows(le.packed, le.scale, conv_npad(le.Cout), le.Cout, conv_kpad(le.Cin), f.fz_we, st);
        if (!rc) rc = launch_scale_cols(net->params[ld.p_kernel].dev, ld.scale, 9, ld.Cout, f.fz_wd, st);
        if (!rc) rc = launch_scale_rows(lp.packed, lp.scale, conv_npad(lp.Cout), lp.Cout, conv_kpad(lp.Cin), f.fz_wp, st);
        if (!rc) rc = launch_pack_split(f.fz_we, le.Cin, le.Cout, st, true);
        if (!rc) rc = launch_pack_split(f.fz_wp, lp.Cin, lp.Cout, st, true);
        if (rc) return rc;
        f.fz_we3 = f.fz_wp3 = nullptr;
        if (band3_block_supported(fused_shape(*net, f, 1))) {
            rc = dev_alloc(*net, (band3_we_shorts(le.Cout) + 1) / 2, &f.fz_we3);
            if (!rc) rc = dev_alloc(*net, (band3_wp_shorts(conv_npad(lp.Cout), le.Cout) + 1) / 2, &f.fz_wp3);
            if (!rc) rc = launch_band3_pack(f.fz_we, le.Cout, le.Cin, conv_kpad(le.Cin), reinterpret_cast<short*>(f.fz_we3), f.fz_wp,
                                            conv_npad(lp.Cout), conv_kpad(lp.Cin), reinterpret_cast<short*>(f.fz_wp3), st);
            if (rc) return rc;
        }
    }
    return SSD_OK;
}

static int finalize_image_slabs(ssd_net* net, int max_batch, hipStream_t st) {
    size_t slab = 0;
    for (auto& f : net->layers) {
        if (!image_kernel_takes(*net, f)) continue;
        const FusedBlockParams p = fused_shape(*net, f, 1);
        for (int b = 1; b <= max_batch; ++b) slab = std::max(slab, image_block_slab_floats(p, b));
    }
    net->img_slabs = nullptr;
    net->img_tickets = nullptr;
    net->slab_bytes = slab * sizeof(float);
    if (slab) {
        float* tk = nullptr;
        int rc = dev_alloc(*net, slab, &net->img_slabs);
        if (!rc) rc = dev_alloc(*net, (size_t)max_batch, &tk);
        if (rc) return rc;
        net->img_tickets = reinterpret_cast<unsigned*>(tk);
        SSD_HIP(hipMemsetAsync(tk, 0, (size_t)max_batch * sizeof(unsigned), st));
    }
    return SSD_OK;
}

static int finalize_arena(ssd_net* net, int max_batch, hipStream_t st) {
    if (net->arena) (void)hipFree(net->arena);
    net->arena = nullptr;
    const bool poison = getenv("SSD_HIP_DEBUG_POISON") != nullptr;
    const size_t gap = poison ? 1024 : 0;
    size_t total = gap;
    for (auto& t : net->tensors) total += align_up(t.per_image * max_batch, 64) + gap;
    SSD_HIP(hipMalloc((void**)&net->arena, total * sizeof(float)));
    net->arena_bytes = total * sizeof(float);
    size_t off = gap;
    for (auto& t : net->tensors) {
        t.dev = net->arena + off;
        off += align_up(t.per_image * max_batch, 64) + gap;
    }
    SSD_HIP(hipMemset(net->arena, poison ? 0xFF : 0, total * sizeof(float)));
    for (auto& t : net->tensors) { t.planes = nullptr; t.planes_live = false; t.plane_only = false; t.planes_np = t.planes_cap = 0; t.plane_stride = 0; }
    if (net->conv_dma)
        for (const auto& l : net->layers) {
            if (l.kind != LK_CONV || l.in < 0 || l.Cin % 32 != 0) continue;
            Tensor& t = net->tensors[l.in];
            if (t.planes) continue;
            t.planes_np = t.planes_cap = net->precision ? 1 : 3;
            t.plane_stride = (long)align_up(t.per_image * max_batch, 64);
            float* pl = nullptr;
            const int rcp = dev_alloc(*net, (size_t)t.planes_np * t.plane_stride / 2 + 64, &pl);
            if (rcp) return rcp;
            t.planes = reinterpret_cast<short*>(pl);
            SSD_HIP(hipMemsetAsync(pl, 0, ((size_t)t.planes_np * t.plane_stride / 2 + 64) * sizeof(float), st));
        }
    net->max_batch = max_batch;
    return SSD_OK;
}

static int finalize_apply_preset(ssd_net* net, int max_batch, bool* image_preset_ok) {
    for (auto& l : net->layers) { l.cfg = -1; l.split_k = 1; }
    size_t ws_need = 0;
    int n_tuned = 0, n_preset = 0;
    for (auto& l : net->layers) {
        if (l.kind != LK_CONV) continue;
        auto it = net->preset.find(l.name);
        if (it == net->preset.end()) { ++n_tuned; continue; }
        int cfg = -1;
        for (int c = 0; c < conv_num_configs(); ++c)
            if (it->second.first == conv_config_name(c)) cfg = c;
        SSD_UNSUPPORTED_IF(cfg >= 0 && conv_config_is_dmah(cfg) && net->precision != 0,
                           "finalize: the table puts layer %s on %s: the two-plane fp16 tiles are admitted in fp32 nets (precision 0) only",
                           l.name.c_str(), conv_config_name(cfg));
        if (cfg >= 0 && conv_config_is_dmah(cfg) && (!net->conv_f16x2 || !l.wh)) cfg = conv_dmah_twin(cfg);
        if (cfg < 0 || !conv_config_allowed(cfg, net->precision)) { ++n_tuned; continue; }
        l.cfg = cfg;
        l.split_k = it->second.second;
        ConvParams p = layer_conv_params(*net, l, max_batch, net->tensors[l.in].dev,
                                         l.out >= 0 ? net->tensors[l.out].dev : nullptr, nullptr,
                                         net->arena, net->arena);
        if (conv_config_is_dmah(cfg)) p.xp_np = 2;
        const bool split_ok = l.split_k == 1 || conv_k_tiles(cfg, p) >= l.split_k;
        if (l.split_k < 1 || !split_ok || !conv_config_valid(cfg, p)) { l.cfg = -1; l.split_k = 1; ++n_tuned; continue; }
        ++n_preset;
        if (l.split_k > 1) ws_need = std::max(ws_need, (size_t)l.split_k * p.M * p.Cout);
    }
    *image_preset_ok = true;
    for (auto& f : net->layers) {
// ... 24 lines not shown
    net->plane_bytes = net->wplane_bytes;
    for (size_t i = 0; i < net->tensors.size(); ++i) {
        Tensor& t = net->tensors[i];
        if (!t.planes) continue;
        const size_t bytes = ((size_t)t.planes_cap * t.plane_stride / 2 + 64) * sizeof(float);
        if (read[i]) { net->plane_bytes += bytes; continue; }
        float* pl = reinterpret_cast<float*>(t.planes);
        net->owned.erase(std::remove(net->owned.begin(), net->owned.end(), pl), net->owned.end());
        (void)hipFree(pl);
        t.planes = nullptr; t.planes_np = t.planes_cap = 0; t.plane_stride = 0;
    }
    return SSD_OK;
}

static void finalize_resolve_f16x2(ssd_net* net) {
    const int nt = (int)net->tensors.size();
    std::vector<char> any(nt, 0), all(nt, 1);
    for (const auto& l : net->layers) {
        if (l.kind != LK_CONV || l.in < 0 || !conv_config_is_dma(l.cfg)) continue;
        any[l.in] = 1;
        if (!conv_config_is_dmah(l.cfg) || !l.wh || !net->conv_f16x2) all[l.in] = 0;
    }
    net->wplane_bytes = 0;
    for (auto& l : net->layers) {
        if (l.kind != LK_CONV) continue;
        if (conv_config_is_dmah(l.cfg) && !(any[l.in] && all[l.in])) l.cfg = conv_dmah_twin(l.cfg);
        if (conv_config_is_dmah(l.cfg)) {
            net->tensors[l.in].planes_np = 2;
            net->wplane_bytes += (conv_f16x2_plane_shorts(l.kh * l.kw * l.Cin, l.Cout) + 1) / 2 * sizeof(float);
        } else if (l.wh) {
            net->owned.erase(std::remove(net->owned.begin(), net->owned.end(), l.wh), net->owned.end());
            (void)hipFree(l.wh);
            l.wh = nullptr;
        }
    }
}

static int finalize_streams(ssd_net* net, int max_batch) {
    size_t total_ws = 0;
    for (auto& l : net->layers)
        if (l.kind == LK_CONV && l.split_k > 1) total_ws += align_up((size_t)l.split_k * max_batch * l.Ho * l.Wo * l.Cout, 64);
    if (total_ws) {
        SSD_HIP(hipMalloc((void**)&net->splitk_layers, total_ws * sizeof(float)));
        size_t o = 0;
        for (auto& l : net->layers)
            if (l.kind == LK_CONV && l.split_k > 1) {
                l.splitk_part = net->splitk_layers + o;
                o += align_up((size_t)l.split_k * max_batch * l.Ho * l.Wo * l.Cout, 64);
            }
    }
    for (int k = 0; k < ssd_net::kSides; ++k) {
        if (!net->side[k]) SSD_HIP(hipStreamCreateWithFlags(&net->side[k], hipStreamNonBlocking));
        if (!net->ev_side_done[k]) SSD_HIP(hipEventCreateWithFlags(&net->ev_side_done[k], hipEventDisableTiming));
    }
    for (auto& l : net->layers)
        if (!l.ev_ready) SSD_HIP(hipEventCreateWithFlags(&l.ev_ready, hipEventDisableTiming));
    return SSD_OK;
}

int ssd_net_finalize(ssd_net* net, int max_batch) {
    SSD_CHECK_ARG(net && max_batch >= 1, "ssd_net_finalize: bad arguments");
    for (const auto& p : net->params)
        if (!p.set) {
            set_error("ssd_net_finalize: parameter '%s' was never set", p.name.c_str());
            return SSD_E_STATE;
        }
    hipStream_t st = nullptr;
    for (float* p : net->owned)
        if (p) (void)hipFree(p);
    net->owned.clear();
    if (net->splitk_layers) (void)hipFree(net->splitk_layers);
    net->splitk_layers = nullptr;
    int rc = SSD_OK;
    for (auto& l : net->layers) {
        l.packed = l.scale = l.shift = nullptr;
        l.wino = nullptr;
        l.wh = nullptr;
        l.splitk_part = nullptr;
        if (l.kind == LK_CONV) rc = finalize_pack_conv(net, l, st);
        if (!rc && (l.kind == LK_CONV || l.kind == LK_DW)) rc = finalize_fold_bn(net, l, st);
        if (rc) return rc;
    }
    rc = finalize_fused_weights(net, st);
    if (!rc) rc = finalize_image_slabs(net, max_batch, st);
    if (!rc) rc = finalize_arena(net, max_batch, st);
    bool image_preset_ok = true;
    if (!rc) rc = finalize_apply_preset(net, max_batch, &image_preset_ok);
    if (!rc && net->n_autotuned) rc = autotune(*net, max_batch, st);
    if (!rc) {
        SSD_HIP(hipStreamSynchronize(st));
        finalize_resolve_f16x2(net);
    }
    if (!rc) rc = finalize_free_unread_planes(net, st);
    if (!rc) rc = finalize_streams(net, max_batch);
    if (rc) return rc;
    if (!image_preset_ok) {
        rc = tune_image_blocks(*net, max_batch, st);
        if (rc) return rc;
        ++net->n_autotuned;
    }
    SSD_HIP(hipDeviceSynchronize());
    net->drop_graphs();
    resolve_routes(*net);
    net->finalized = true;
    return tune_launch_mode(net, max_batch);
}

long ssd_net_get_tuning(const ssd_net* net, char* buf, size_t cap) {
    if (!net) return SSD_E_INVALID;
    std::string out;
    for (const auto& l : net->layers)
        if (l.kind == LK_CONV && l.cfg >= 0)
            out += l.name + " " + conv_config_name(l.cfg) + " " + std::to_string(l.split_k) + "\n";
    for (const auto& l : net->layers)
        if (l.img_choice >= 0 && image_kernel_takes(*net, l)) out += l.name + " image " + std::to_string(l.img_choice) + "\n";
    if (net->finalized && net->use_graph_auto && net->launch_raced)
        out += std::string("__launch graph ") + (net->use_graph ? "1" : "0") + "\n";
    if (buf && cap > out.size()) memcpy(buf, out.c_str(), out.size() + 1);
    return (long)out.size();
}

int ssd_net_memory_bytes(const ssd_net* net, size_t out[4]) {
    SSD_CHECK_ARG(net != nullptr && out != nullptr, "ssd_net_memory_bytes: NULL argument");
    SSD_CHECK_ARG(net->finalized, "ssd_net_memory_bytes: net is not finalized");
    out[0] = net->arena_bytes;
    out[1] = net->plane_bytes;
    out[2] = net->slab_bytes;
    size_t sk = net->splitk_floats;
    for (const auto& l : net->layers)
        if (l.kind == LK_CONV && l.split_k > 1) sk += align_up((size_t)l.split_k * net->max_batch * l.Ho * l.Wo * l.Cout, 64);
    out[3] = sk * sizeof(float);
    return SSD_OK;
}

int ssd_net_tuning_stats(const ssd_net* net, int* from_table, int* timed) {
    SSD_CHECK_ARG(net != nullptr, "ssd_net_tuning_stats: net is NULL");
    if (from_table) *from_table = net->n_preset;
    if (timed) *timed = net->n_autotuned;
    return SSD_OK;
}

int ssd_net_set_tuning(ssd_net* net, const char* text) {
    SSD_CHECK_ARG(net && text, "ssd_net_set_tuning: NULL argument");
    net->preset.clear();
    std::string s(text);
    size_t pos = 0;
    while (pos < s.size()) {
        size_t e = s.find('\n', pos);
        if (e == std::string::npos) e = s.size();
        const std::string line = s.substr(pos, e - pos);
        pos = e + 1;
        char name[128], cfg[128];
        int split = 1;
        if (line.empty() || line[0] == '#') continue;
        const bool flag = sscanf(line.c_str(), "%127s %127s %d", name, cfg, &split) == 3 &&
                          (std::string(cfg) == "image" || std::string(cfg) == "graph");
        if (sscanf(line.c_str(), "%127s %127s %d", name, cfg, &split) == 3 && split >= (flag ? 0 : 1) && split <= 64)
            net->preset[name] = {cfg, split};
    }
    net->finalized = false;
    return SSD_OK;
}

int ssd_net_num_priors(const ssd_net* net) { return net ? net->num_priors : 0; }
int ssd_net_feature_map_size(const ssd_net* net, int level) {
    return (net && level >= 0 && level < (int)net->fmap.size()) ? net->fmap[level] : 0;
}

static void plan_steps(ssd_net& net) {
    for (auto& t : net.tensors) t.planes_live = false;
    for (const auto& l : net.layers)
        if (l.kind == LK_CONV && l.in >= 0 && conv_config_is_dma(l.cfg) && net.tensors[l.in].planes && layer_runs(l))
            net.tensors[l.in].planes_live = true;
    {
        const std::vector<char> only = plane_only_candidates(net, [&](int i) { return conv_config_is_dma(net.layers[i].cfg); });
        for (size_t t = 0; t < net.tensors.size(); ++t) net.tensors[t].plane_only = only[t] && net.tensors[t].planes_live;
    }
    const bool overlap = net.overlap_heads && !net.timing && net.side[0];
    const int nl = (int)net.layers.size();
    const bool tail_on_side = net.tail_on_side;
    auto producer_of = [&](int i, int tensor) {
        for (int j = i - 1; j >= 0; --j)
            if ((net.layers[j].out == tensor || net.layers[j].e_out == tensor) && layer_runs(net.layers[j])) return j;
        return -1;
    };
    std::vector<int> sid(nl, -1);
    std::vector<int> order;
    order.reserve(nl);
    if (overlap) {
        int split = -1;
        for (int j = 0; j < nl && split < 0; ++j) {
            const Layer& h = net.layers[j];
            if (h.side == 2 && layer_runs(h)) split = producer_of(j, h.in);
        }
        std::vector<char> placed(nl, 0);
        auto place = [&](int i, int stream) { order.push_back(i); placed[i] = 1; sid[i] = stream; };
        auto place_small_heads = [&](int out_tensor) {
            for (int j = 0; j < nl; ++j) {
                const Layer& c = net.layers[j];
                if (!placed[j] && c.side == 2 && c.in == out_tensor && layer_runs(c)) place(j, 1);
            }
        };
        for (int i = 0; i < nl; ++i) {
            const Layer& l = net.layers[i];
            if (!l.side && l.kind != LK_SOFTMAX && (split < 0 || i <= split)) place(i, -1);
        }
        for (int i = 0; i < nl; ++i) {
            if (net.layers[i].side != 1) continue;
            const int pr = producer_of(i, net.layers[i].in);
            if (pr >= 0 && !placed[pr]) place(pr, -1);
            place(i, tail_on_side ? -1 : 0);
        }
        if (split >= 0) place_small_heads(net.layers[split].out);
        for (int i = 0; i < nl; ++i) {
            const Layer& l = net.layers[i];
// ... 140 lines not shown
        net->nms_ws_bytes = need;
        net->nms_ws_batch = ws_batch;
        net->nms_ws_total = max_per_class;
    }
    hipStream_t st = (hipStream_t)stream;
    SSD_CHECK_ARG(var != nullptr, "ssd_net_predict: variances pointer is NULL");
    const float v4[4] = {var[0], var[1], var[2], var[3]};
    union { float f; intptr_t i; } k1{}, k2{};
    k1.f = iou_thr; k2.f = score_thr;
    std::vector<const void*> key = {image_dev, priors_dev, boxes_dev, labels_dev, scores_dev, valid_dev,
                                    (const void*)(intptr_t)B, (const void*)(intptr_t)max_total,
                                    (const void*)k1.i, (const void*)k2.i, (const void*)(intptr_t)(cfg ? 3 : 2)};
    for (int i = 0; i < 4; ++i) { union { float f; intptr_t i; } k{}; k.f = v4[i]; key.push_back((const void*)k.i); }
    if (cfg) {
        union { float f; intptr_t i; } ks{};
        ks.f = cfg->sigma;
        for (const int v : {cfg->method, cfg->class_agnostic != 0 ? 1 : 0, cfg->max_per_class, cfg->clip_boxes})
            key.push_back((const void*)(intptr_t)v);
        key.push_back((const void*)ks.i);
    }
    const bool fused_sm = net->fuse_softmax && decode_nms_fused_ok(L) && N >= 1 && net->nms_ws_batch >= B;
    int rc = run_graphed(net, key, st, [&]() {
        int r = forward_impl(net, image_dev, B, net->deltas, net->probs, st, fused_sm);
        if (r) return r;
        if (cfg && fused_sm)
            return decode_nms_fused_cfg(net->deltas, net->probs, priors_dev, v4, B, N, L, cfg, boxes_dev, labels_dev, scores_dev,
                                        valid_dev, net->nms_ws, net->nms_ws_bytes, net->nms_ws_batch, st);
        if (cfg)
            return ssd_decode_nms_cfg(net->deltas, net->probs, priors_dev, v4, B, N, L, cfg, boxes_dev, labels_dev, scores_dev,
                                      valid_dev, nullptr, net->nms_ws, net->nms_ws_bytes, (void*)st);
        if (fused_sm)
            return decode_nms_fused(net->deltas, net->probs, priors_dev, v4, B, N, L, max_total, max_total, iou_thr, score_thr,
                                    boxes_dev, labels_dev, scores_dev, valid_dev, net->nms_ws, net->nms_ws_bytes, net->nms_ws_batch, st);
        return ssd_decode_nms(net->deltas, net->probs, priors_dev, v4, B, N, L, max_total, max_total, iou_thr,
                              score_thr, boxes_dev, labels_dev, scores_dev, valid_dev, nullptr, net->nms_ws,
                              net->nms_ws_bytes, (void*)st);
    });
    if (rc && fused_sm && net->nms_ws) {
        (void)hipDeviceSynchronize();
        (void)hipMemset(net->nms_ws, 0, net->nms_ws_bytes);
    }
    if (!rc && net->timing && !net->timing_events.empty())
        (void)hipEventRecord(net->timing_events.back().back(), st);
    return rc;
}

int ssd_net_predict(ssd_net* net, const float* image_dev, int B, const float* priors_dev, const float* var,
                    int max_total, float iou_thr, float score_thr, float* boxes_dev, float* labels_dev,
                    float* scores_dev, int* valid_dev, void* stream) {
    return predict_impl(net, image_dev, B, priors_dev, var, max_total, iou_thr, score_thr, nullptr, boxes_dev, labels_dev,
                        scores_dev, valid_dev, stream);
}

int ssd_net_predict_cfg(ssd_net* net, const float* image_dev, int B, const float* priors_dev, const float* var,
                        const ssd_nms_config* cfg, float* boxes_dev, float* labels_dev, float* scores_dev,
                        int* valid_dev, void* stream) {
    SSD_CHECK_ARG(cfg != nullptr, "ssd_net_predict_cfg: config is NULL");
    return predict_impl(net, image_dev, B, priors_dev, var, cfg->max_total, cfg->iou_threshold, cfg->score_threshold, cfg,
                        boxes_dev, labels_dev, scores_dev, valid_dev, stream);
}

struct OptionSpec {
    const char* name;
    bool ssd_net::*flag;
    int ssd_net::*num;
    int lo, hi, refinalize;
};
static const OptionSpec kOptions[] = {
    {"fuse_blocks", &ssd_net::fuse_blocks, nullptr, 0, 1, 0},
    {"precision", nullptr, &ssd_net::precision, 0, 1, 1},
    {"fuse_band", nullptr, &ssd_net::fuse_band, 0, 2, 0},
    {"fuse_image", nullptr, &ssd_net::fuse_image, 0, 2, 0},
    {"lanes_hint", nullptr, &ssd_net::lanes_hint, 1, 8, 0},
    {"tail_on_side", &ssd_net::tail_on_side, nullptr, 0, 1, 0},
    {"image_split", &ssd_net::image_split, nullptr, 0, 1, 1},
    {"image_ticket", &ssd_net::image_ticket, nullptr, 0, 1, 0},
    {"fuse_softmax", &ssd_net::fuse_softmax, nullptr, 0, 1, 0},
    {"fuse_dwproj", &ssd_net::fuse_dwproj, nullptr, 0, 1, 0},
    {"overlap_heads", &ssd_net::overlap_heads, nullptr, 0, 1, 0},
    {"use_wino", &ssd_net::use_wino, nullptr, 0, 1, 2},
    {"image_v2", &ssd_net::image_v2, nullptr, 0, 1, 0},
    {"conv_dma", &ssd_net::conv_dma, nullptr, 0, 1, 1},
    {"conv_f16x2", &ssd_net::conv_f16x2, nullptr, 0, 1, 1},
    {"plane_only", &ssd_net::plane_only, nullptr, 0, 1, 0},
    {"use_graph", &ssd_net::use_graph, nullptr, 0, 1, 0},
};

int ssd_net_set_option(ssd_net* net, const char* name, int value) {
    SSD_CHECK_ARG(net && name, "ssd_net_set_option: NULL argument");
    const std::string n(name);
    const OptionSpec* o = nullptr;
    for (const OptionSpec& k : kOptions)
        if (n == k.name) o = &k;
    if (!o) {
        set_error("ssd_net_set_option: unknown option '%s'", name);
        return SSD_E_INVALID;
    }
    if (n == "precision") SSD_CHECK_ARG(value == 0 || value == 1, "ssd_net_set_option: precision must be 0 (fp32) or 1 (bf16)");
    if (n == "use_graph") {
        if (value && net->graphs_unsafe && net->overlap_heads) {
            set_error("ssd_net_set_option: use_graph 1 needs overlap_heads 0 with GPU_MAX_HW_QUEUES < 4 (hipGraph capture of the forked step crashes in the runtime; a single in-order stream replays fine)");
            return SSD_E_UNSUPPORTED;
        }
        net->use_graph_auto = false;
    }
    const int v = o->flag ? value != 0 : std::min(std::max(value, o->lo), o->hi);
    const int old = o->flag ? (int)(net->*o->flag) : net->*o->num;
    if (o->flag) net->*o->flag = v != 0;
    else net->*o->num = v;
    if (o->refinalize == 2 || (o->refinalize == 1 && v != old)) net->finalized = false;
    net->drop_graphs();
    resolve_routes(*net);
    if (n == "fuse_softmax" && net->nms_ws) {
        (void)hipDeviceSynchronize();
        SSD_HIP(hipMemset(net->nms_ws, 0, net->nms_ws_bytes));
    }
    return SSD_OK;
}

int ssd_net_set_timing(ssd_net* net, int enabled) {
    SSD_CHECK_ARG(net != nullptr, "ssd_net_set_timing: net is NULL");
    net->timing = enabled != 0;
    net->steps.clear();
    return SSD_OK;
}

int ssd_net_read_timing(ssd_net* net, float* ms_sum_out, int* forwards_out) {
    SSD_CHECK_ARG(net && ms_sum_out && forwards_out, "ssd_net_read_timing: NULL argument");
    const size_t nl = net->layers.size();
    for (size_t i = 0; i <= nl; ++i) ms_sum_out[i] = 0.f;
    SSD_HIP(hipDeviceSynchronize());
    for (auto& ev : net->timing_events) {
        for (size_t i = 0; i < nl; ++i) {
            float ms = 0.f;
            if (hipEventElapsedTime(&ms, ev[i], ev[i + 1]) == hipSuccess) ms_sum_out[i] += ms;
        }
        float ms = 0.f;
        if (hipEventQuery(ev[nl + 1]) == hipSuccess && hipEventElapsedTime(&ms, ev[nl], ev[nl + 1]) == hipSuccess)
            ms_sum_out[nl] += ms;
        for (auto e : ev) (void)hipEventDestroy(e);
    }
    *forwards_out = (int)net->timing_events.size();
    net->timing_events.clear();
    return SSD_OK;
}

long ssd_net_fetch_activation(ssd_net* net, const char* layer, float* host_out, size_t cap) {
    if (!net || !layer) return SSD_E_INVALID;
    auto it = net->tensor_index.find(layer);
    if (it == net->tensor_index.end()) {
        set_error("ssd_net_fetch_activation: unknown tensor '%s'", layer);
        return SSD_E_INVALID;
    }
    const Tensor& t = net->tensors[it->second];
    const size_t n = t.per_image * (size_t)net->last_batch;
    if (!host_out) return (long)n;
    if (cap < n) {
        set_error("ssd_net_fetch_activation: buffer holds %zu floats, need %zu", cap, n);
        return SSD_E_INVALID;
    }
    ScopedDev joined;
    const float* src = t.dev;
    if (t.plane_only && n) {
        SSD_HIP(hipMalloc((void**)&joined.p, n * sizeof(float)));
        SSD_HIP(hipDeviceSynchronize());
        const int rc = launch_join_planes(t.planes, (long)n, t.C, t.planes_np, t.plane_stride, joined.p, nullptr);
        if (rc) return rc;
        src = joined.p;
    }
    if (hipDeviceSynchronize() != hipSuccess || hipMemcpy(host_out, src, n * sizeof(float), hipMemcpyDeviceToHost) != hipSuccess) {
        set_error("ssd_net_fetch_activation: copy failed");
        return SSD_E_HIP;
    }
    return (long)n;
}

long ssd_net_fetch_planes(ssd_net* net, const char* layer, float* host_out, size_t cap, int* planes_out) {
    if (!net || !layer) return SSD_E_INVALID;
    auto it = net->tensor_index.find(layer);
    if (it == net->tensor_index.end()) {
        set_error("ssd_net_fetch_planes: unknown tensor '%s'", layer);
        return SSD_E_INVALID;
    }
    const Tensor& t = net->tensors[it->second];
    if (planes_out) *planes_out = t.planes_np;
    if (!t.planes || !t.planes_live) return 0;
    const size_t n = t.per_image * (size_t)net->last_batch;
    if (!host_out) return (long)n;
    if (cap < n) {
        set_error("ssd_net_fetch_planes: buffer holds %zu floats, need %zu", cap, n);
        return SSD_E_INVALID;
    }
    ScopedDev tmp;
    SSD_HIP(hipMalloc((void**)&tmp.p, n * sizeof(float)));
    SSD_HIP(hipDeviceSynchronize());
    const int rc = launch_join_planes(t.planes, (long)n, t.C, t.planes_np, t.plane_stride, tmp.p, nullptr);
    if (rc) return rc;
    if (hipDeviceSynchronize() != hipSuccess || hipMemcpy(host_out, tmp.p, n * sizeof(float), hipMemcpyDeviceToHost) != hipSuccess) {
        set_error("ssd_net_fetch_planes: copy failed");
        return SSD_E_HIP;
    }
    return (long)n;
}

int ssd_net_num_layers(const ssd_net* net) { return net ? (int)net->layers.size() : 0; }
const char* ssd_net_layer_name(const ssd_net* net, int i) {
    return (net && i >= 0 && i < (int)net->layers.size()) ? net->layers[i].name.c_str() : "";
}
const char* ssd_net_layer_kind(const ssd_net* net, int i) {
    return (net && i >= 0 && i < (int)net->layers.size()) ? kKindName[net->layers[i].kind] : "";
}
const char* ssd_net_layer_config(const ssd_net* net, int i) {
    if (!net || i < 0 || i >= (int)net->layers.size()) return "";
    static thread_local char buf[64];
    const Layer& l = net->layers[i];
    static const char* const kFamily[][2] = {{"", ""}, {"", ""}, {"stem_split", "stem_bf16"}, {"dwproj", "dwproj_bf16"}, {"tile", "tile"},
                                             {"band", "band"}, {"band3", "band_bf16"}, {"image", "image_bf16"}, {"image_split", "image_bf16"}};
    if (l.kind == LK_FUSED) return kFamily[l.route][net->precision ? 1 : 0];
    if (l.kind != LK_CONV) return "";
    if (l.split_k > 1) snprintf(buf, sizeof(buf), "%s/s%d", conv_config_name(l.cfg), l.split_k);
    else snprintf(buf, sizeof(buf), "%s", conv_config_name(l.cfg));
    return buf;
}
static double algorithmic_flops(const Layer& l, int B) {
    const double px = (double)B * l.Ho * l.Wo;
    if (l.kind == LK_CONV) return 2.0 * px * l.kh * l.kw * l.Cin * l.Cout;
    if (l.kind == LK_DW) return 2.0 * px * 9 * l.Cout;
    return 0;
}
double ssd_net_layer_flops(const ssd_net* net, int i, int B) {
    if (!net || i < 0 || i >= (int)net->layers.size()) return 0;
    const Layer& l = net->layers[i];
    if (!layer_runs(l)) return 0;
    if (l.kind != LK_FUSED) return algorithmic_flops(l, B);
    double f = 0;
    for (int m : {l.f_expand, l.f_dw, l.f_project})
        if (m >= 0) f += algorithmic_flops(net->layers[m], B);
    return f;
}
double ssd_net_layer_executed_flops(const ssd_net* net, int i, int B) {
    if (!net || i < 0 || i >= (int)net->layers.size()) return 0;
    const Layer& l = net->layers[i];
    if (!layer_runs(l)) return 0;
    if (l.kind == LK_CONV && conv_config_family(l.cfg) == CF_WINO)
        return 2.0 * B * ((l.Ho + 1) / 2) * ((l.Wo + 1) / 2) * 16.0 * l.Cin * l.Cout;
    return ssd_net_layer_flops(net, i, B);
}
double ssd_net_layer_bytes(const ssd_net* net, int i, int B) {
    if (!net || i < 0 || i >= (int)net->layers.size()) return 0;
    const Layer& l = net->layers[i];
    if (!layer_runs(l)) return 0;
    if (l.kind == LK_FUSED)
        return 4.0 * B * ((double)l.H * l.W * l.Cin + (double)l.Ho * l.Wo * l.Cout);
    if (l.kind == LK_SOFTMAX) return 2.0 * 4.0 * B * net->num_priors * net->L;
    double b = 4.0 * B * ((double)l.H * l.W * l.Cin + (double)l.Ho * l.Wo * l.Cout);
    if (l.res >= 0) b += 4.0 * B * (double)l.Ho * l.Wo * l.Cout;
    if (l.kind == LK_CONV) b += 4.0 * l.kh * l.kw * l.Cin * l.Cout;
    if (l.kind == LK_DW) b += 4.0 * 9 * l.Cout;
    return b;
}

int ssd_net_profile_layers(ssd_net* net, const float* image_dev, int B, int reps, float* ms_out, void* stream) {
    SSD_CHECK_ARG(net && image_dev && ms_out && reps >= 1, "ssd_net_profile_layers: bad arguments");
    if (!net->finalized) {
        set_error("ssd_net_profile_layers: call ssd_net_finalize() first");
        return SSD_E_STATE;
    }
    SSD_CHECK_ARG(B >= 1 && B <= net->max_batch, "ssd_net_profile_layers: bad batch %d", B);
    hipStream_t st = (hipStream_t)stream;
    const int N = net->num_priors, L = net->L;
    ScopedDev sd, spr;
    SSD_HIP(hipMalloc((void**)&sd.p, (size_t)B * N * 4 * sizeof(float)));
    SSD_HIP(hipMalloc((void**)&spr.p, (size_t)B * N * L * sizeof(float)));
    float *d = sd.p, *pr = spr.p;
    int rc = forward_impl(net, image_dev, B, d, pr, st);
    ScopedEvent se0, se1;
    SSD_HIP(hipEventCreate(&se0.e));
    SSD_HIP(hipEventCreate(&se1.e));
    hipEvent_t e0 = se0.e, e1 = se1.e;
    for (size_t i = 0; i < net->layers.size() && !rc; ++i) {
        (void)hipEventRecord(e0, st);
        for (int r = 0; r < reps && !rc && layer_runs(net->layers[i]); ++r)
            rc = run_layer(*net, net->layers[i], B, d, pr, st);
        (void)hipEventRecord(e1, st);
        (void)hipEventSynchronize(e1);
        float ms = 0.f;
        (void)hipEventElapsedTime(&ms, e0, e1);
        ms_out[i] = ms / reps;
    }
    return rc;
}

}
```

tf-ssd_amd/models/_net.py:

```python
import ctypes
import os
import re

import numpy as np
import torch

import ssd_hip as _h

_TABLE_OPTIONS = ("use_wino", "image_split", "conv_dma")
_REFINALIZE_OPTIONS = ("precision", "image_split", "use_wino", "conv_dma", "conv_f16x2")
_STALE_WARNED = set()


class _LayerProxy(object):

    def __init__(self, model, name):
        self._model = model
        self.name = name

    @property
    def trainable(self):
        return self._model._is_trainable(self.name)

    @trainable.setter
    def trainable(self, value):
        self._model._set_trainable(self.name, bool(value))


class SSDModel(object):

    def __init__(self, backbone, hyper_params, max_batch=None, precision="fp32"):
        if precision not in ("fp32", "bf16"):
            raise ValueError("precision must be 'fp32' or 'bf16', got %r" % (precision,))
        self.precision = precision
        self.backbone = backbone
        self.hyper_params = hyper_params
        self.img_size = int(hyper_params["img_size"])
        self.total_labels = int(hyper_params["total_labels"])
        n_ars = [len(a) for a in hyper_params["aspect_ratios"]]
        arr = (ctypes.c_int * len(n_ars))(*n_ars)
        lib = _h.lib()
        self._net = lib.ssd_net_create(_h.MOBILENET_V2 if backbone == "mobilenet_v2" else _h.VGG16,
                                       self.img_size, len(n_ars), arr, self.total_labels)
        if not self._net:
            raise ValueError("ssd_net_create: %s" % lib.ssd_last_error().decode())
        self.param_specs = []
        for i in range(lib.ssd_net_num_params(self._net)):
            name = lib.ssd_net_param_name(self._net, i).decode()
            rank = lib.ssd_net_param_rank(self._net, i)
            shp = lib.ssd_net_param_shape(self._net, i)
            self.param_specs.append((name, tuple(shp[j] for j in range(rank))))
        self.num_priors = lib.ssd_net_num_priors(self._net)
        fm = [lib.ssd_net_feature_map_size(self._net, l) for l in range(len(n_ars))]
        if list(fm) != [int(f) for f in hyper_params["feature_map_shapes"]]:
            raise ValueError("feature_map_shapes %s do not match the %s graph at img_size %d (%s)" % (
                hyper_params["feature_map_shapes"], backbone, self.img_size, fm))
        self._max_batch = max_batch
        self._finalized_for = 0
        self._weights_set = False
        self._weights_version = 0
        self._options = {}
        if precision == "bf16":
            self.set_option("precision", 1)

    def __del__(self):
        try:
            if getattr(self, "_comm_stream", None) is not None:
                _h.free_stream(self._comm_stream)
                self._comm_stream = None
            if getattr(self, "_net", None):
                _h.lib().ssd_net_destroy(self._net)
                self._net = None
        except Exception:
            pass

    def set_weights(self, weights):
        lib = _h.lib()
        _h.device()
        shapes = dict(self.param_specs)
        for name, value in weights.items():
            if name not in shapes:
                raise ValueError("unknown parameter %r" % name)
            a = np.ascontiguousarray(np.asarray(value, dtype=np.float32))
            if tuple(a.shape) != shapes[name]:
                raise ValueError("parameter %r has shape %s, expected %s" % (name, a.shape, shapes[name]))
            _h.check(lib.ssd_net_set_param(self._net, name.encode(), a.ctypes.data_as(_h.c_float_p), a.size),
                     "set_weights")
        self._weights_set = True
        self._finalized_for = 0
        self._weights_version += 1

    def clone(self):
        m = SSDModel(self.backbone, self.hyper_params, self._max_batch, precision=self.precision)
# ... 126 lines not shown
            magic = f.read(8)
        if magic == b"\x89HDF\r\n\x1a\n":
            from utils import h5_reader
            w = h5_reader.load_keras_weights(path)
        elif magic[:2] == b"PK":
            with np.load(path) as z:
                w = {k: z[k] for k in z.files}
        else:
            raise ValueError("%s is neither an HDF5 (Keras) nor an .npz weights file" % path)
        shapes = dict(self.param_specs)
        if by_name:
            w = {k: v for k, v in w.items() if k in shapes}
        else:
            missing = [k for k in shapes if k not in w]
            extra = [k for k in w if k not in shapes]
            if missing or extra:
                raise ValueError("weights file %s does not match the %s graph: %d missing (e.g. %s), %d unexpected "
                                 "(e.g. %s); use by_name=True for a partial load" % (
                                     path, self.backbone, len(missing), missing[:2], len(extra), extra[:2]))
        self.set_weights(w)

    def _ensure(self, B):
        if not self._weights_set:
            raise RuntimeError("model has no weights: call set_weights()/load_weights() first")
        want = max(B, self._max_batch or 0)
        if self._finalized_for < want:
            self._finalize(want)

    def _finalize(self, want):
        import tuning
        lib = _h.lib()
        key = tuning.table_key(self.backbone, self.img_size, self.total_labels, self.hyper_params["aspect_ratios"], want)
        if self.precision != "fp32":
            key += "_" + self.precision
        opts = tuning.options_key({k: v for k, v in self._options.items() if k in _TABLE_OPTIONS})
        source, text, path = "autotune", None, None
        explicit = getattr(self, "_tuning_explicit", None)
        cache = os.environ.get("SSD_HIP_TUNE_CACHE")
        if cache:
            props = torch.cuda.get_device_properties(torch.cuda.current_device())
            dev = "%s_cu%d" % (str(getattr(props, "gcnArchName", "gpu")).split(":")[0], props.multi_processor_count)
            path = os.path.join(cache, "%s_%s_%s%s.tune" % (key, dev, lib.ssd_build_id().decode(), ("_" + opts) if opts else ""))
        if explicit is not None:
            source, text = "explicit", explicit
        elif path and os.path.exists(path):
            with open(path) as f:
                source, text = "cache", f.read()
        elif not opts and os.environ.get("SSD_HIP_IGNORE_SHIPPED", "0") != "1" and tuning.load_shipped(key) is not None:
            source, text = "shipped", tuning.load_shipped(key)
        elif tuning.memo_get(key, opts) is not None:
            source, text = "memo", tuning.memo_get(key, opts)
        _h.check(lib.ssd_net_set_tuning(self._net, tuning.body(text or "").encode()), "ssd_net_set_tuning")
        if text is None and os.environ.get("SSD_HIP_AUTOTUNE", "1") == "0":
            raise RuntimeError("no tuning table for %s and SSD_HIP_AUTOTUNE=0 (tables: %s)" % (key, tuning.SHIPPED_DIR))
        _h.check(lib.ssd_net_finalize(self._net, want), "ssd_net_finalize")
        self._finalized_for = want
        a, b = ctypes.c_int(0), ctypes.c_int(0)
        _h.check(lib.ssd_net_tuning_stats(self._net, ctypes.byref(a), ctypes.byref(b)), "ssd_net_tuning_stats")
        table = self.get_tuning()
        hdr = tuning.header(text or "")
        this_build = lib.ssd_build_id().decode()
        stale = bool(text) and hdr.get("build") not in (None, this_build)
        self.tuning_info = {"key": key, "source": source, "table_sha16": tuning.sha16(table), "layers_from_table": a.value,
                            "choices_timed_on_device": b.value, "reproducible": b.value == 0,
                            "table_build": hdr.get("build"), "this_build": this_build, "stale": stale}
        if stale and os.environ.get("SSD_HIP_WARN_STALE_TABLE", "1") != "0" and key not in _STALE_WARNED:
            _STALE_WARNED.add(key)
            import warnings
            warnings.warn("kernel table %s (%s) was measured on build %s, this library is %s: choices stay valid and "
                          "reproducible but may be slower than a re-measured table (tools/make_tuning_tables.py)" % (
                              key, source, hdr.get("build"), this_build))
        if explicit is None:
            tuning.memo_put(key, opts, table)
        if path and not os.path.exists(path):
            os.makedirs(cache, exist_ok=True)
            tmp = "%s.%d.tmp" % (path, os.getpid())
            with open(tmp, "w") as f:
                f.write(tuning.with_header(table, key=key, build=lib.ssd_build_id().decode()))
            os.replace(tmp, path)

    def memory_summary(self):
        out = (ctypes.c_size_t * 4)()
        _h.check(_h.lib().ssd_net_memory_bytes(self._net, out), "ssd_net_memory_bytes")
        return {"arena": int(out[0]), "planes": int(out[1]), "image_slabs": int(out[2]), "splitk_slabs": int(out[3])}

    def set_tuning(self, text):
        self._tuning_explicit = text
        self._finalized_for = 0

    def __call__(self, images):
        x = _h.to_dev(images)
        if x.dim() != 4 or x.shape[1] != self.img_size or x.shape[2] != self.img_size or x.shape[3] != 3:
            raise ValueError("expected images [B,%d,%d,3], got %s" % (self.img_size, self.img_size, tuple(x.shape)))
        B = x.shape[0]
        self._ensure(max(B, 1))
        dev = x.device
        deltas = torch.empty((B, self.num_priors, 4), dtype=torch.float32, device=dev)
        probs = torch.empty((B, self.num_priors, self.total_labels), dtype=torch.float32, device=dev)
        _h.check(_h.lib().ssd_net_forward(self._net, _h.ptr(x), B, _h.ptr(deltas), _h.ptr(probs), _h.stream()),
                 "ssd_net_forward")
        self._last_input = x
        return deltas, probs

    def predict(self, x, batch_size=32, steps=None, verbose=0):
        outs = ([], [])
        n = x.shape[0]
        for i in range(0, n, batch_size):
            d, p = self(x[i:i + batch_size])
            outs[0].append(d.cpu().numpy())
            outs[1].append(p.cpu().numpy())
        return np.concatenate(outs[0], 0), np.concatenate(outs[1], 0)

    def get_tuning(self):
        lib = _h.lib()
        n = lib.ssd_net_get_tuning(self._net, None, 0)
        buf = ctypes.create_string_buffer(n + 1)
        lib.ssd_net_get_tuning(self._net, buf, n + 1)
        return buf.value.decode()

    def fetch_activation(self, name):
        lib = _h.lib()
        n = lib.ssd_net_fetch_activation(self._net, name.encode(), None, 0)
        if n < 0:
            raise ValueError(lib.ssd_last_error().decode())
        a = np.empty((n,), np.float32)
        got = lib.ssd_net_fetch_activation(self._net, name.encode(), a.ctypes.data_as(_h.c_float_p), a.size)
        if got < 0:
            raise RuntimeError(lib.ssd_last_error().decode())
        return a

    def fetch_planes(self, name):
        lib = _h.lib()
        npl = ctypes.c_int(0)
        n = lib.ssd_net_fetch_planes(self._net, name.encode(), None, 0, ctypes.byref(npl))
        if n < 0:
            raise ValueError(lib.ssd_last_error().decode())
        if n == 0:
            return None, npl.value
        a = np.empty((n,), np.float32)
        got = lib.ssd_net_fetch_planes(self._net, name.encode(), a.ctypes.data_as(_h.c_float_p), a.size, ctypes.byref(npl))
        if got < 0:
            raise RuntimeError(lib.ssd_last_error().decode())
        return a, npl.value

    def layers(self, B):
        lib = _h.lib()
        out = []
        for i in range(lib.ssd_net_num_layers(self._net)):
            out.append({"name": lib.ssd_net_layer_name(self._net, i).decode(),
                        "kind": lib.ssd_net_layer_kind(self._net, i).decode(),
                        "config": lib.ssd_net_layer_config(self._net, i).decode(),
                        "flops": lib.ssd_net_layer_flops(self._net, i, B),
                        "executed_flops": lib.ssd_net_layer_executed_flops(self._net, i, B),
                        "bytes": lib.ssd_net_layer_bytes(self._net, i, B)})
        return out

    def predict_on_device(self, images, priors, variances, max_total=200, iou_threshold=0.5,
                          score_threshold=0.5, nms_config=None):
        x = _h.to_dev(images)
        B = x.shape[0]
        self._ensure(max(B, 1))
        pri = _h.to_dev(priors)
        dev = x.device
        boxes = torch.empty((B, max_total, 4), dtype=torch.float32, device=dev)
        labels = torch.empty((B, max_total), dtype=torch.float32, device=dev)
        scores = torch.empty((B, max_total), dtype=torch.float32, device=dev)
        valid = torch.empty((B,), dtype=torch.int32, device=dev)
# ... 297 lines not shown
```

tf-ssd_amd/ssd_hip.py:

```python
import ctypes
import os
import sys


def configure_serving(lanes=3):
    if "GPU_MAX_HW_QUEUES" in os.environ:
        return os.environ["GPU_MAX_HW_QUEUES"] == str(lanes)
    t = sys.modules.get("torch")
    try:
        if t is not None and t.cuda.is_initialized():
            return False
    except Exception:
        return False
    os.environ["GPU_MAX_HW_QUEUES"] = str(int(lanes))
    return True


if os.environ.get("SSD_HIP_HW_QUEUES", "").isdigit() and int(os.environ["SSD_HIP_HW_QUEUES"]) > 0:
    configure_serving(int(os.environ["SSD_HIP_HW_QUEUES"]))

import numpy as np
import torch

_HERE = os.path.dirname(os.path.abspath(__file__))
# ... 134 lines not shown
    "ssd_png_encode_bound": (ctypes.c_size_t, [ctypes.c_int, ctypes.c_int]),
    "ssd_png_encode_workspace_bytes": (ctypes.c_size_t, [vp, ctypes.c_int]),
    "ssd_png_encode": (ctypes.c_int, [vp, ctypes.c_size_t, vp, vp, ctypes.c_int, vp, ctypes.c_size_t, vp, vp, ctypes.c_size_t, vp]),
    "ssd_png_encode_host": (ctypes.c_int, [vp, ctypes.c_int, ctypes.c_int, ctypes.c_int, vp, ctypes.c_size_t,
                                            ctypes.POINTER(ctypes.c_size_t)]),
    "ssd_png_parse": (ctypes.c_int, [vp, ctypes.c_size_t, ctypes.POINTER(PngInfo)]),
    "ssd_png_idat": (ctypes.c_int, [vp, ctypes.c_size_t, ctypes.POINTER(PngInfo), vp, ctypes.c_size_t]),
    "ssd_png_decode_host": (ctypes.c_int, [ctypes.POINTER(PngInfo), vp, ctypes.c_size_t, vp, ctypes.c_size_t]),
    "ssd_png_decode_workspace_bytes": (ctypes.c_size_t, [vp, ctypes.c_int]),
    "ssd_png_decode": (ctypes.c_int, [vp, ctypes.c_size_t, vp, vp, ctypes.c_int, vp, ctypes.c_size_t, vp, ctypes.c_size_t, vp]),
    "ssd_png_inflate": (ctypes.c_int, [vp, ctypes.c_size_t, vp, vp, ctypes.c_int, vp, vp]),
    "ssd_png_inflate_host": (ctypes.c_int, [vp, ctypes.c_size_t, vp, ctypes.c_size_t, ctypes.c_longlong, c_int_p]),
    "ssd_jpeg_scan_plan": (ctypes.c_int, [vp, ctypes.c_size_t, ctypes.POINTER(JpegInfo), ctypes.POINTER(JpegScanPlan), vp, ctypes.c_size_t]),
    "ssd_jpeg_entropy_decode_subseq": (ctypes.c_int, [vp, ctypes.c_size_t, ctypes.POINTER(JpegInfo), vp, ctypes.c_size_t, ctypes.c_int]),
    "ssd_jpeg_unpack_slots": (ctypes.c_int, [ctypes.c_longlong, ctypes.c_int, ctypes.c_int]),
    "ssd_jpeg_unpack_workspace_bytes": (ctypes.c_size_t, [vp, ctypes.c_int, ctypes.c_int]),
    "ssd_jpeg_unpack": (ctypes.c_int, [vp, ctypes.c_size_t, vp, vp, ctypes.c_int, ctypes.c_int, vp, ctypes.c_size_t, vp, vp,
                                        ctypes.c_size_t, vp]),
    "ssd_image_mean": (ctypes.c_int, [vp] + [ctypes.c_int] * 4 + [vp, vp, vp]),
    "ssd_augment_geometry": (ctypes.c_int, [vp] + [ctypes.c_int] * 6 + [vp, vp, vp, vp]),
    "ssd_augment_color": (ctypes.c_int, [vp] + [ctypes.c_int] * 3 + [vp, vp, vp, vp]),
    "ssd_augment_plan": (ctypes.c_int, [vp, vp, vp] + [ctypes.c_int] * 4 + [ctypes.c_ulonglong] + [vp] * 7),
    "ssd_augment_mosaic_plan": (ctypes.c_int, [vp, vp, vp] + [ctypes.c_int] * 4 + [ctypes.c_ulonglong] + [ctypes.c_float] * 3 +
                                [ctypes.c_int] * 2 + [vp] * 5),
    "ssd_augment_mosaic_pixels": (ctypes.c_int, [vp] + [ctypes.c_int] * 3 + [vp, c_float_p, vp, vp]),
    "ssd_image_minmax_workspace_bytes": (ctypes.c_size_t, [ctypes.c_int]),
    "ssd_image_minmax": (ctypes.c_int, [vp] + [ctypes.c_int] * 4 + [vp, vp, ctypes.c_size_t, vp]),
    "ssd_draw_detections": (ctypes.c_int, [vp, vp] + [ctypes.c_int] * 4 + [vp, vp, vp, vp, ctypes.c_int, ctypes.c_int, vp,
                                           ctypes.c_int, vp, ctypes.c_int, ctypes.c_int, vp, vp]),
    "ssd_draw_bounding_boxes": (ctypes.c_int, [vp] + [ctypes.c_int] * 4 + [vp, ctypes.c_int, vp, ctypes.c_int, vp, vp]),
    "ssd_loss_workspace_bytes": (ctypes.c_size_t, [ctypes.c_int, ctypes.c_int]),
    "ssd_loss": (ctypes.c_int, [vp, vp, vp, vp, ctypes.c_int, ctypes.c_int, ctypes.c_int, ctypes.c_float,
                                ctypes.c_float, vp, vp, vp, vp, vp, vp, ctypes.c_float, vp, ctypes.c_size_t, vp]),
    "ssd_focal_loss_tile": (ctypes.c_int, [ctypes.c_int, c_int_p]),
    "ssd_focal_loss_workspace_bytes": (ctypes.c_size_t, [ctypes.c_int, ctypes.c_int, ctypes.c_int]),
    "ssd_focal_loss": (ctypes.c_int, [vp, vp, vp, vp, ctypes.c_int, ctypes.c_int, ctypes.c_int, ctypes.c_float,
                                      ctypes.c_float, ctypes.c_float, vp, vp, vp, vp, vp, vp, ctypes.c_float, vp,
                                      ctypes.c_size_t, vp]),
    "ssd_iou_loc_loss_tile": (ctypes.c_int, []),
    "ssd_iou_loc_loss_workspace_bytes": (ctypes.c_size_t, [ctypes.c_int, ctypes.c_int]),
    "ssd_iou_loc_loss": (ctypes.c_int, [vp, ctypes.POINTER(ctypes.c_float), vp, vp, ctypes.c_int, ctypes.c_int, ctypes.c_int,
                                        ctypes.c_float, vp, vp, vp, ctypes.c_float, vp, ctypes.c_size_t, vp]),
    "ssd_loss_config_bytes": (ctypes.c_size_t, []),
    "ssd_same_pads": (ctypes.c_int, [ctypes.c_int] * 4 + [c_int_p, c_int_p]),
    "ssd_conv_out_size": (ctypes.c_int, [ctypes.c_int] * 6),
    "ssd_conv_packed_weight_floats": (ctypes.c_size_t, [ctypes.c_int] * 4),
    "ssd_conv_pack_weights": (ctypes.c_int, [vp] + [ctypes.c_int] * 4 + [vp, vp]),
    "ssd_conv2d": (ctypes.c_int, [ctypes.POINTER(ConvDesc), vp, vp, vp, vp, vp, vp,
                                  ctypes.c_long, ctypes.c_long, vp]),
    "ssd_conv_num_configs": (ctypes.c_int, []),
    "ssd_conv_config_name": (ctypes.c_char_p, [ctypes.c_int]),
    "ssd_conv2d_ex": (ctypes.c_int, [ctypes.POINTER(ConvDesc), vp, vp, vp, vp, vp, vp,
                                     ctypes.c_long, ctypes.c_long, ctypes.c_int, ctypes.c_int, vp, vp]),
    "ssd_split_planes": (ctypes.c_int, [vp, ctypes.c_long, ctypes.c_int, ctypes.c_int, vp, ctypes.c_long, vp]),
    "ssd_join_planes": (ctypes.c_int, [vp, ctypes.c_long, ctypes.c_int, ctypes.c_int, ctypes.c_long, vp, vp]),
    "ssd_conv2d_planes": (ctypes.c_int, [ctypes.POINTER(ConvDesc), vp, ctypes.c_int, ctypes.c_long, vp, vp, vp, vp, vp,
                                         ctypes.c_long, ctypes.c_long, vp, ctypes.c_long, ctypes.c_int, ctypes.c_int, vp, vp]),
    "ssd_conv_f16x2_weight_bytes": (ctypes.c_size_t, [ctypes.c_int] * 4),
    "ssd_conv_pack_weights_f16x2": (ctypes.c_int, [vp] + [ctypes.c_int] * 4 + [vp, c_int_p, vp]),
    "ssd_conv2d_planes_f16x2": (ctypes.c_int, [ctypes.POINTER(ConvDesc), vp, ctypes.c_long, vp, vp, ctypes.c_int, vp, vp, vp, vp,
                                               ctypes.c_long, ctypes.c_long, vp, ctypes.c_long, ctypes.c_int, ctypes.c_int, vp, vp]),
    "ssd_conv_wino_weight_floats": (ctypes.c_size_t, [ctypes.c_int, ctypes.c_int]),
    "ssd_conv_wino_pack_weights": (ctypes.c_int, [vp, ctypes.c_int, ctypes.c_int, vp, vp]),
    "ssd_conv_wino_num_configs": (ctypes.c_int, []),
    "ssd_conv2d_wino": (ctypes.c_int, [ctypes.POINTER(ConvDesc), vp, vp, vp, vp, vp, ctypes.c_long, ctypes.c_long,
                                       ctypes.c_int, ctypes.c_int, vp, vp]),
    "ssd_dwconv3x3": (ctypes.c_int, [vp] + [ctypes.c_int] * 9 + [vp, vp, vp, ctypes.c_int, vp, vp]),
    "ssd_maxpool2d": (ctypes.c_int, [vp] + [ctypes.c_int] * 10 + [vp, vp]),
    "ssd_l2norm": (ctypes.c_int, [vp, ctypes.c_long, ctypes.c_int, vp, vp, vp]),
    "ssd_softmax": (ctypes.c_int, [vp, ctypes.c_long, ctypes.c_int, vp, vp]),
    "ssd_net_create": (vp, [ctypes.c_int, ctypes.c_int, ctypes.c_int, c_int_p, ctypes.c_int]),
    "ssd_net_destroy": (None, [vp]),
    "ssd_net_num_params": (ctypes.c_int, [vp]),
    "ssd_net_param_name": (ctypes.c_char_p, [vp, ctypes.c_int]),
    "ssd_net_param_rank": (ctypes.c_int, [vp, ctypes.c_int]),
    "ssd_net_param_shape": (c_int_p, [vp, ctypes.c_int]),
    "ssd_net_set_param": (ctypes.c_int, [vp, ctypes.c_char_p, c_float_p, ctypes.c_size_t]),
    "ssd_net_get_param": (ctypes.c_int, [vp, ctypes.c_char_p, c_float_p, ctypes.c_size_t]),
    "ssd_net_finalize": (ctypes.c_int, [vp, ctypes.c_int]),
    "ssd_net_get_tuning": (ctypes.c_long, [vp, ctypes.c_char_p, ctypes.c_size_t]),
    "ssd_net_set_tuning": (ctypes.c_int, [vp, ctypes.c_char_p]),
    "ssd_net_tuning_stats": (ctypes.c_int, [vp, ctypes.POINTER(ctypes.c_int), ctypes.POINTER(ctypes.c_int)]),
    "ssd_net_memory_bytes": (ctypes.c_int, [vp, ctypes.POINTER(ctypes.c_size_t)]),
    "ssd_build_id": (ctypes.c_char_p, []),
    "ssd_stream_create": (vp, [ctypes.c_int]),
    "ssd_stream_create_masked": (vp, [ctypes.POINTER(ctypes.c_uint), ctypes.c_int]),
    "ssd_stream_destroy": (ctypes.c_int, [vp]),
    "ssd_net_regularization_loss": (ctypes.c_int, [vp, c_float_p]),
    "ssd_net_train_set_buckets": (ctypes.c_int, [vp, ctypes.c_int, ctypes.POINTER(ctypes.c_long)]),
    "ssd_net_train_wait_bucket": (ctypes.c_int, [vp, ctypes.c_int, vp]),
    "ssd_net_num_priors": (ctypes.c_int, [vp]),
    "ssd_net_feature_map_size": (ctypes.c_int, [vp, ctypes.c_int]),
    "ssd_net_forward": (ctypes.c_int, [vp, vp, ctypes.c_int, vp, vp, vp]),
    "ssd_net_predict": (ctypes.c_int, [vp, vp, ctypes.c_int, vp, c_float_p, ctypes.c_int,
                                       ctypes.c_float, ctypes.c_float, vp, vp, vp, vp, vp]),
    "ssd_net_predict_cfg": (ctypes.c_int, [vp, vp, ctypes.c_int, vp, c_float_p, ctypes.POINTER(NmsConfig), vp, vp, vp, vp, vp]),
    "ssd_net_fetch_activation": (ctypes.c_long, [vp, ctypes.c_char_p, c_float_p, ctypes.c_size_t]),
    "ssd_net_fetch_planes": (ctypes.c_long, [vp, ctypes.c_char_p, c_float_p, ctypes.c_size_t, c_int_p]),
    "ssd_net_num_layers": (ctypes.c_int, [vp]),
    "ssd_net_layer_name": (ctypes.c_char_p, [vp, ctypes.c_int]),
    "ssd_net_layer_kind": (ctypes.c_char_p, [vp, ctypes.c_int]),
    "ssd_net_layer_config": (ctypes.c_char_p, [vp, ctypes.c_int]),
    "ssd_net_layer_flops": (ctypes.c_double, [vp, ctypes.c_int, ctypes.c_int]),
    "ssd_net_layer_bytes": (ctypes.c_double, [vp, ctypes.c_int, ctypes.c_int]),
    "ssd_net_layer_executed_flops": (ctypes.c_double, [vp, ctypes.c_int, ctypes.c_int]),
    "ssd_net_set_option": (ctypes.c_int, [vp, ctypes.c_char_p, ctypes.c_int]),
    "ssd_net_set_timing": (ctypes.c_int, [vp, ctypes.c_int]),
    "ssd_net_read_timing": (ctypes.c_int, [vp, c_float_p, c_int_p]),
    "ssd_net_profile_layers": (ctypes.c_int, [vp, vp, ctypes.c_int, ctypes.c_int, c_float_p, vp]),
    "ssd_net_train_begin": (ctypes.c_int, [vp, ctypes.c_int]),
    "ssd_net_trainable_floats": (ctypes.c_size_t, [vp]),
    "ssd_net_trainable_offset": (ctypes.c_long, [vp, ctypes.c_char_p]),
    "ssd_net_train_forward_backward": (ctypes.c_int, [vp, vp, ctypes.c_int, vp, vp, ctypes.c_float, ctypes.c_float,
                                                      vp, vp, vp, vp]),
    "ssd_net_train_forward_backward_cfg": (ctypes.c_int, [vp, vp, ctypes.c_int, vp, vp, ctypes.POINTER(LossConfig), vp, vp, vp, vp]),
    "ssd_net_adam_step": (ctypes.c_int, [vp, vp, ctypes.c_float, ctypes.c_float, ctypes.c_float, ctypes.c_float,
                                         ctypes.c_float, vp]),
    "ssd_net_optimizer_step": (ctypes.c_int, [vp, vp, ctypes.POINTER(Optimizer), ctypes.c_float, ctypes.c_float, vp]),
    "ssd_net_optimizer_reset": (ctypes.c_int, [vp]),
    "ssd_net_optimizer_get_state": (ctypes.c_long, [vp, ctypes.c_char_p, c_float_p, ctypes.c_size_t]),
    "ssd_net_optimizer_set_state": (ctypes.c_int, [vp, ctypes.c_char_p, c_float_p, ctypes.c_size_t]),
    "ssd_net_train_set_steps": (ctypes.c_int, [vp, ctypes.c_long]),
    "ssd_net_set_trainable": (ctypes.c_int, [vp, ctypes.c_char_p, ctypes.c_int]),
    "ssd_net_get_trainable": (ctypes.c_int, [vp, ctypes.c_char_p]),
    "ssd_net_train_plan": (ctypes.c_int, [vp, ctypes.c_int, c_int_p]),
    "ssd_net_train_steps": (ctypes.c_long, [vp]),
    "ssd_net_train_matrix_flops": (ctypes.c_int, [vp, ctypes.POINTER(ctypes.c_double)]),
    "ssd_net_train_fetch": (ctypes.c_long, [vp, ctypes.c_char_p, ctypes.c_int, c_float_p, ctypes.c_size_t]),
    "ssd_conv_wgrad_num_configs": (ctypes.c_int, []),
    "ssd_conv_wgrad_workspace_floats": (ctypes.c_size_t, [ctypes.POINTER(ConvDesc), ctypes.c_int]),
    "ssd_conv2d_wgrad_ex": (ctypes.c_int, [ctypes.POINTER(ConvDesc), vp, vp, ctypes.c_int, ctypes.c_int, ctypes.c_int,
                                           vp, vp, ctypes.c_size_t, vp]),
    "ssd_dwconv3x3_backward": (ctypes.c_int, [vp, vp, vp] + [ctypes.c_int] * 8 + [vp, vp, vp, ctypes.c_size_t, vp]),
}

MAX_IMAGE_SIDE = 16384
RESIZE_DESC_DTYPE = np.dtype([("src_offset", "<i8"), ("tmp_offset", "<i8")] + [(n, "<i4") for n in (
    "H", "W", "h_bounds", "h_k", "h_ksize", "v_bounds", "v_k", "v_ksize")])
assert RESIZE_DESC_DTYPE.itemsize == ctypes.sizeof(ResizeDesc) == 48
IMAGE_DESC_DTYPE = np.dtype([("src_offset", "<i8"), ("H", "<i4"), ("W", "<i4")])
assert IMAGE_DESC_DTYPE.itemsize == 16
JPEG_DESC_DTYPE = np.dtype([("coef_offset", "<i8"), ("quant_offset", "<i8"), ("plane_offset", "<i8")] + [(n, "<i4") for n in (
    "kind", "H", "W", "components", "h_samp", "v_samp", "block_start", "item_start")])
assert JPEG_DESC_DTYPE.itemsize == 56 and ctypes.sizeof(JpegInfo) == 504
JPEG_ENC_DESC_DTYPE = np.dtype([(n, "<i8") for n in ("src_offset", "coef_offset", "quant_offset", "plane_offset")] + [
    (n, "<i4") for n in ("H", "W", "h_samp", "v_samp", "block_start", "item_start")])
assert JPEG_ENC_DESC_DTYPE.itemsize == 56
JPEG_HEADER_BYTES = 623
JPEG_PACK_DESC_DTYPE = np.dtype([("coef_offset", "<i8"), ("header_offset", "<i8")] + [
    (n, "<i4") for n in ("H", "W", "h_samp", "v_samp", "block_start", "reserved")])
assert JPEG_PACK_DESC_DTYPE.itemsize == 40
PNG_DESC_DTYPE = np.dtype([("src_offset", "<i8")] + [(n, "<i4") for n in ("H", "W", "filter", "seg_start", "row_start", "reserved")])
assert PNG_DESC_DTYPE.itemsize == 32
PNG_SEGMENT_BYTES = 16384
PNG_FILTERS = {"none": 0, "sub": 1, "up": 2, "average": 3, "paeth": 4, "adaptive": 5}
PNG_DEC_DESC_DTYPE = np.dtype([(n, "<i8") for n in ("src_offset", "palette_offset", "chain_offset", "dst_offset", "raw_offset")] + [
    (n, "<i4") for n in ("H", "W", "depth", "color_type", "chains", "chain_start", "row_start", "reserved")])
assert PNG_DEC_DESC_DTYPE.itemsize == 72 and ctypes.sizeof(PngInfo) == 832
PNG_SIGNATURE = b"\x89PNG\r\n\x1a\n"
PNG_INFLATE_DESC_DTYPE = np.dtype([(n, "<i8") for n in ("zlib_offset", "zlib_bytes", "dst_offset", "chain_offset", "row_bytes")] + [
    ("H", "<i4"), ("reserved", "<i4")])
assert PNG_INFLATE_DESC_DTYPE.itemsize == 48
PNG_INFLATE_MAX_STREAM = 1 << 20
PNG_INFLATE_STATUS = {"header": 0x0001, "block_type": 0x0002, "stored": 0x0004, "symbols": 0x0008, "repeat": 0x0010,
                      "oversubscribed": 0x0020, "incomplete": 0x0040, "no_end": 0x0080, "symbol": 0x0100, "distance": 0x0200,
                      "input": 0x0400, "output": 0x0800, "adler": 0x1000, "trailing": 0x2000, "filter": 0x4000}
# ... 174 lines not shown
```

Before: 63100.

## Add two-plane fp16 form for image-split fused MobileNetV2 blocks using static bounds

```diff
diff --git a/include/ssd_hip.h b/include/ssd_hip.h
--- a/include/ssd_hip.h
+++ b/include/ssd_hip.h
@@ -470,6 +470,11 @@
 int ssd_net_set_tuning(ssd_net* net, const char* text);
 int ssd_net_tuning_stats(const ssd_net* net, int* from_table, int* timed);
 int ssd_net_memory_bytes(const ssd_net* net, size_t out[4]);
+size_t ssd_net_image_f16x2_bytes(const ssd_net* net);
+float ssd_net_tensor_bound(const ssd_net* net, const char* tensor);
+int ssd_block_output_interval(const float* w, int n, int k, int ld, const float* scale, const float* shift, const double* res_lo,
+                              const double* res_hi, double* lo, double* hi);
+int ssd_f16x2_input_exp(float bound, int* s);
 const char* ssd_build_id(void);
 int ssd_net_num_priors(const ssd_net* net);
 int ssd_net_feature_map_size(const ssd_net* net, int level);
@@ -492,6 +497,7 @@
 const char* ssd_net_layer_name(const ssd_net* net, int i);
 const char* ssd_net_layer_kind(const ssd_net* net, int i);
 const char* ssd_net_layer_config(const ssd_net* net, int i);
+int ssd_net_layer_image_form(const ssd_net* net, int i, int B);
 double ssd_net_layer_flops(const ssd_net* net, int i, int B);
 double ssd_net_layer_bytes(const ssd_net* net, int i, int B);
 double ssd_net_layer_executed_flops(const ssd_net* net, int i, int B);
diff --git a/tf-ssd_amd/csrc/ssd_bf16x3.h b/tf-ssd_amd/csrc/ssd_bf16x3.h
--- a/tf-ssd_amd/csrc/ssd_bf16x3.h
+++ b/tf-ssd_amd/csrc/ssd_bf16x3.h
@@ -101,6 +101,22 @@
     return r;
 }
 template <int NP>
+__device__ __forceinline__ BP<NP> splitN_scaled(const b3_f32x4 a, const b3_f32x4 b, const float scale) {
+    if constexpr (NP == 2) {
+        uint4 h, l;
+        split_h2(a[0] * scale, a[1] * scale, h.x, l.x);
+        split_h2(a[2] * scale, a[3] * scale, h.y, l.y);
+        split_h2(b[0] * scale, b[1] * scale, h.z, l.z);
+        split_h2(b[2] * scale, b[3] * scale, h.w, l.w);
+        BP<NP> r;
+        r.p[0] = __builtin_bit_cast(bf16x8, h);
+        r.p[1] = __builtin_bit_cast(bf16x8, l);
+        return r;
+    } else {
+        return splitN<NP>(a, b);
+    }
+}
+template <int NP>
 __device__ __forceinline__ b3_f32x4 mmaN(const BP<NP>& w, const BP<NP>& x, b3_f32x4 acc) {
     if constexpr (NP == 2) {
         const f16x8 wh = __builtin_bit_cast(f16x8, w.p[0]), wl = __builtin_bit_cast(f16x8, w.p[1]);
diff --git a/tf-ssd_amd/csrc/ssd_conv.h b/tf-ssd_amd/csrc/ssd_conv.h
--- a/tf-ssd_amd/csrc/ssd_conv.h
+++ b/tf-ssd_amd/csrc/ssd_conv.h
@@ -71,6 +71,7 @@
     int e_planes_np;
     int planes_only;
     int form2;
+    float f16_xs, f16_es, f16_ps;
 };
 struct StemParams {
     const float* x;
@@ -174,7 +175,7 @@
 void mfma3_tile(int i, int* BM, int* BN);
 int dmah_tile_index(int j);
 int launch_absmax_bits(const float* packed, int K, int Cout, unsigned* absmax_bits_dev, hipStream_t st);
-int launch_pack_f16x2(const float* packed, int K, int Cout, int k, short* planes, hipStream_t st);
+int launch_pack_f16x2(const float* packed, int K, int Cout, int k, short* planes, hipStream_t st, bool row_major = false);
 inline int conv_f16x2_weight_exp(unsigned absmax_bits) {
     float wmax;
     std::memcpy(&wmax, &absmax_bits, sizeof(float));
diff --git a/tf-ssd_amd/csrc/ssd_convdma.hip b/tf-ssd_amd/csrc/ssd_convdma.hip
--- a/tf-ssd_amd/csrc/ssd_convdma.hip
+++ b/tf-ssd_amd/csrc/ssd_convdma.hip
@@ -305,7 +305,7 @@
                                                          const float scale, short* __restrict__ out) {
     for (long e = (long)blockIdx.x * 256 + threadIdx.x; e < total; e += (long)gridDim.x * 256) {
         const long n = e / Kpad;
-        const long d = plane_elem(n, (int)(e - n * Kpad), Npad);
+        const long d = Npad ? plane_elem(n, (int)(e - n * Kpad), Npad) : e;
         unsigned h, l;
         split_h2(w[e] * scale, 0.f, h, l);
         out[d] = (short)(h & 0xffffu);
@@ -392,11 +392,11 @@
     SSD_LAUNCH_CHECK();
     return SSD_OK;
 }
-int launch_pack_f16x2(const float* packed, int K, int Cout, int k, short* planes, hipStream_t st) {
+int launch_pack_f16x2(const float* packed, int K, int Cout, int k, short* planes, hipStream_t st, bool row_major) {
     const long total = (long)conv_kpad(K) * conv_npad(Cout);
     if (total == 0) return SSD_OK;
     const int blocks = (int)((total + 255) / 256 < 8192 ? (total + 255) / 256 : 8192);
-    hipLaunchKernelGGL(pack_f16x2_kernel, dim3(blocks), dim3(256), 0, st, packed, total, conv_kpad(K), conv_npad(Cout), ldexpf(1.f, k), planes);
+    hipLaunchKernelGGL(pack_f16x2_kernel, dim3(blocks), dim3(256), 0, st, packed, total, conv_kpad(K), row_major ? 0 : conv_npad(Cout), ldexpf(1.f, k), planes);
     SSD_LAUNCH_CHECK();
     return SSD_OK;
 }
diff --git a/tf-ssd_amd/csrc/ssd_imgblock.hip b/tf-ssd_amd/csrc/ssd_imgblock.hip
--- a/tf-ssd_amd/csrc/ssd_imgblock.hip
+++ b/tf-ssd_amd/csrc/ssd_imgblock.hip
@@ -681,6 +681,8 @@
     SSD_CHECK_ARG(!p.planes_only || !p.tickets, "image block: plane-only outputs combine by the second launch only");
     SSD_CHECK_ARG((p.Ce / kIC) % p.groups == 0, "image block: %d groups do not divide Ce/16 = %d", p.groups, p.Ce / kIC);
     SSD_CHECK_ARG(p.groups == 1 || p.slabs, "image block: %d groups need the slab workspace", p.groups);
+    SSD_UNSUPPORTED_IF(p.bf16 == 2 && !(p.form2 && !p.tickets && image_block2_supported(p)),
+                       "image block: the two-plane fp16 form has no kernel for Cin=%d Ce=%d Cout=%d %dx%d at %d groups", p.Cin, p.Ce, p.Cout, p.H, p.W, p.groups);
     if (p.bf16 == 3 && image_lds_bytes(*c, p, p.groups) > 160 * 1024) p.bf16 = 0;
     const size_t lds = image_lds_bytes(*c, p, p.groups);
     SSD_UNSUPPORTED_IF(lds > 160 * 1024, "image block: needs %zu B of LDS", lds);
diff --git a/tf-ssd_amd/csrc/ssd_imgblock2.hip b/tf-ssd_amd/csrc/ssd_imgblock2.hip
--- a/tf-ssd_amd/csrc/ssd_imgblock2.hip
+++ b/tf-ssd_amd/csrc/ssd_imgblock2.hip
@@ -89,7 +89,7 @@
         for (int ks = 0; ks < KS; ++ks) {
             const f32x4 lo = real[t] ? *reinterpret_cast<const f32x4*>(xp + ks * 32) : f32x4{0.f, 0.f, 0.f, 0.f};
             const f32x4 hi = real[t] ? *reinterpret_cast<const f32x4*>(xp + ks * 32 + 4) : f32x4{0.f, 0.f, 0.f, 0.f};
-            xs[t][ks] = splitN<NP>(lo, hi);
+            xs[t][ks] = splitN_scaled<NP>(lo, hi, p.f16_xs);
         }
     }
     for (int u = tid; u < 11 * (CeG / 4); u += NTH) {
@@ -127,7 +127,7 @@
         f32x4 ea[T];
         const f32x4 sh = *reinterpret_cast<const f32x4*>(ps_l + j * PCH);
 #pragma unroll
-        for (int t = 0; t < T; ++t) ea[t] = sh;
+        for (int t = 0; t < T; ++t) ea[t] = NP == 2 ? f32x4{0.f, 0.f, 0.f, 0.f} : sh;
         const short* wl = we_l + pb * NBE * 512;
 #pragma unroll
         for (int ks = 0; ks < KS; ++ks) {
@@ -141,6 +141,7 @@
 #pragma unroll
         for (int t = 0; t < T; ++t) {
             f32x4 v = ea[t];
+            if constexpr (NP == 2) v = v * p.f16_es + sh;
 #pragma unroll
             for (int e = 0; e < 4; ++e) v[e] = __builtin_amdgcn_fmed3f(v[e], 0.0f, relu_hi[t]);
             *reinterpret_cast<f32x4*>(ew + t * ROW) = v;
@@ -183,7 +184,7 @@
     auto project = [&](const f32x4 (&a0)[TO], const f32x4 (&a1)[TO]) {
         BP<NP> d[TO];
 #pragma unroll
-        for (int t = 0; t < TO; ++t) d[t] = splitN<NP>(a0[t], a1[t]);
+        for (int t = 0; t < TO; ++t) d[t] = splitN_scaled<NP>(a0[t], a1[t], kF16x2ActScale);
 #pragma unroll
         for (int ni = 0; ni < NT; ++ni) {
             BP<NP> wa;
@@ -232,6 +233,12 @@
         }
     }
 
+    if constexpr (NP == 2) {
+#pragma unroll
+        for (int t = 0; t < TO; ++t)
+#pragma unroll
+            for (int ni = 0; ni < NT; ++ni) acc[t][ni] = acc[t][ni] * p.f16_ps;
+    }
     const long img_off = (long)img * (Ho * Wo) * p.Cout;
     if (G == 1) {
 #pragma unroll
@@ -268,10 +275,12 @@
 typedef void (*image2_kernel_t)(const FusedBlockParams);
 struct Image2Cfg {
     int cin, nt, nw, t, h, w, stride;
-    image2_kernel_t fn1, fn3;
+    image2_kernel_t fn1, fn3, fn2;
 };
-#define I2CFG(CIN, NT, NW, T, H, W, LOOP) {CIN, NT, NW, T, H, W, 1, mbv2_image16v2_kernel<CIN, NT, NW, T, H, W, 1, LOOP>, mbv2_image16v2_kernel<CIN, NT, NW, T, H, W, 3, LOOP>}
-#define I2CFG2(CIN, NT, NW, T, H, W, LOOP) {CIN, NT, NW, T, H, W, 2, mbv2_image16v2_kernel<CIN, NT, NW, T, H, W, 1, LOOP, 2>, mbv2_image16v2_kernel<CIN, NT, NW, T, H, W, 3, LOOP, 2>}
+#define I2CFG(CIN, NT, NW, T, H, W, LOOP) {CIN, NT, NW, T, H, W, 1, mbv2_image16v2_kernel<CIN, NT, NW, T, H, W, 1, LOOP>, mbv2_image16v2_kernel<CIN, NT, NW, T, H, W, 3, LOOP>, \
+                                           mbv2_image16v2_kernel<CIN, NT, NW, T, H, W, 2, LOOP>}
+#define I2CFG2(CIN, NT, NW, T, H, W, LOOP) {CIN, NT, NW, T, H, W, 2, mbv2_image16v2_kernel<CIN, NT, NW, T, H, W, 1, LOOP, 2>, mbv2_image16v2_kernel<CIN, NT, NW, T, H, W, 3, LOOP, 2>, \
+                                            mbv2_image16v2_kernel<CIN, NT, NW, T, H, W, 2, LOOP, 2>}
 const Image2Cfg kImage2[] = {
     I2CFG(64, 4, 8, 3, 19, 19, 1),
     I2CFG(64, 6, 8, 3, 19, 19, 1),
@@ -284,7 +293,7 @@
 
 size_t image2_lds_bytes(const Image2Cfg& c, const FusedBlockParams& p, int G) {
     const int P = c.w + 1, npix = c.nw * 16 * c.t, NE = npix + 2 * P + 2, row = c.stride == 2 ? 20 : (c.t & 1) ? 24 : 20;
-    const int np = p.bf16 == 3 ? 3 : 1, ks = c.cin / 32;
+    const int np = p.bf16 == 3 ? 3 : p.bf16 == 2 ? 2 : 1, ks = c.cin / 32;
     const size_t w = (size_t)(2 * np * ks + np * c.nt) * 1024;
     const int pairs = p.Ce / (2 * kC), cmax = ((pairs + G - 1) / G) * 2 * kC;
     return ((size_t)2 * NE * row + (size_t)11 * cmax) * sizeof(float) + w;
@@ -322,7 +331,7 @@
     SSD_CHECK_ARG(p.we3 && p.wp3, "image block: the bf16 forms need the weights' bf16 planes");
     const size_t lds = image2_lds_bytes(*c, p, p.groups);
     SSD_UNSUPPORTED_IF(lds > 160 * 1024, "image block (second form): needs %zu B of LDS", lds);
-    const image2_kernel_t fn = p.bf16 == 3 ? c->fn3 : c->fn1;
+    const image2_kernel_t fn = p.bf16 == 3 ? c->fn3 : p.bf16 == 2 ? c->fn2 : c->fn1;
     if (lds > 64 * 1024)
         SSD_HIP(hipFuncSetAttribute((const void*)fn, hipFuncAttributeMaxDynamicSharedMemorySize, (int)lds));
     hipLaunchKernelGGL(fn, dim3((unsigned)((long)p.B * p.groups)), dim3(c->nw * 64), lds, st, p);
diff --git a/tf-ssd_amd/csrc/ssd_net.h b/tf-ssd_amd/csrc/ssd_net.h
--- a/tf-ssd_amd/csrc/ssd_net.h
+++ b/tf-ssd_amd/csrc/ssd_net.h
@@ -36,6 +36,8 @@
     int planes_cap = 0;
     bool planes_live = false;
     bool plane_only = false;
+    std::vector<double> blo, bhi;
+    float bound = -1.f;
 };
 
 struct Layer {
@@ -68,6 +70,8 @@
     float* splitk_part = nullptr;
     float *fz_we = nullptr, *fz_wd = nullptr, *fz_wp = nullptr;
     float *fz_we3 = nullptr, *fz_wp3 = nullptr;
+    float *fz_weh = nullptr, *fz_wph = nullptr;
+    int f16_ke = 0, f16_kp = 0, f16_s = 0;
     int side = 0;
     hipEvent_t ev_ready = nullptr;
 };
@@ -128,6 +132,7 @@
     bool image_v2 = true;
     bool conv_dma = true;
     bool conv_f16x2 = true;
+    bool image_f16x2 = true;
     bool plane_only = true;
     bool image_ticket = false;
     float* img_slabs = nullptr;
@@ -138,6 +143,7 @@
     float* arena = nullptr;
     size_t arena_bytes = 0, plane_bytes = 0, slab_bytes = 0;
     size_t wplane_bytes = 0;
+    size_t iplane_bytes = 0;
     float* splitk_ws = nullptr;
     size_t splitk_floats = 0;
     float* deltas = nullptr;
diff --git a/tf-ssd_amd/csrc/ssd_net.hip b/tf-ssd_amd/csrc/ssd_net.hip
--- a/tf-ssd_amd/csrc/ssd_net.hip
+++ b/tf-ssd_amd/csrc/ssd_net.hip
@@ -368,6 +368,16 @@
         p.slabs = net.img_slabs;
         p.tickets = net.image_ticket && !p.bf16 ? net.img_tickets : nullptr;
         if (f.route == RT_IMAGE_SPLIT) { p.bf16 = 3; p.tickets = nullptr; }
+        if (f.route == RT_IMAGE_SPLIT && net.image_f16x2 && net.image_v2 && f.fz_weh && f.fz_wph) {
+            FusedBlockParams q = p;
+            q.bf16 = 2;
+            q.we3 = reinterpret_cast<const short*>(f.fz_weh);
+            q.wp3 = reinterpret_cast<const short*>(f.fz_wph);
+            q.f16_xs = ldexpf(1.f, f.f16_s);
+            q.f16_es = ldexpf(1.f, -(f.f16_s + f.f16_ke));
+            q.f16_ps = ldexpf(1.f, -(8 + f.f16_kp));
+            if (image_block2_supported(q)) return q;
+        }
     }
     return p;
 }
@@ -580,7 +590,10 @@
         for (int choice = 0; choice < nchoice && !rc; ++choice) {
             f.img_choice = choice;
             resolve_routes(net);
-            if (choice == 2 && !image_block_split_fits(fused_params(net, f, B))) continue;
+            if (choice == 2) {
+                const FusedBlockParams fp = fused_params(net, f, B);
+                if (fp.bf16 != 2 && !image_block_split_fits(fp)) continue;
+            }
             for (int trial = 0; trial < 4 && !rc; ++trial) {
                 (void)hipEventRecord(se0.e, st);
                 for (int r = 0; r < 4 && !rc; ++r)
@@ -1052,6 +1065,114 @@
     return SSD_OK;
 }
 
+int ssd_block_output_interval(const float* w, int n, int k, int ld, const float* scale, const float* shift, const double* res_lo,
+                              const double* res_hi, double* lo, double* hi) {
+    SSD_CHECK_ARG(w && lo && hi && n >= 0 && k >= 0 && ld >= k && (res_lo == nullptr) == (res_hi == nullptr), "ssd_block_output_interval: bad arguments");
+    bool finite = true;
+    for (int r = 0; r < n; ++r) {
+        double neg = 0.0, pos = 0.0;
+        const float s = scale ? scale[r] : 1.f;
+        for (int c = 0; c < k; ++c) {
+            const float v = w[(size_t)r * ld + c] * s;
+            finite = finite && std::isfinite(v);
+            if (v < 0.f) neg += v; else pos += v;
+        }
+        const double h = shift ? (double)shift[r] : 0.0;
+        lo[r] = 6.0 * neg + h + (res_lo ? res_lo[r] : 0.0);
+        hi[r] = 6.0 * pos + h + (res_hi ? res_hi[r] : 0.0);
+        finite = finite && std::isfinite(lo[r]) && std::isfinite(hi[r]);
+    }
+    return finite ? 1 : 0;
+}
+int ssd_f16x2_input_exp(float bound, int* s) {
+    if (s) *s = 0;
+    if (!(bound >= 0.f) || !std::isfinite(bound)) return 0;
+    if (bound == 0.f) return 0;
+    int e = 0;
+    const float f = std::frexp(bound, &e);
+    const int v = f == 0.5f ? 16 - e : 15 - e;
+    if (v < -12 || v > 12) return 0;
+    if (s) *s = v;
+    return 1;
+}
+
+static int finalize_tensor_bounds(ssd_net* net, hipStream_t st) {
+    for (auto& t : net->tensors) { t.blo.clear(); t.bhi.clear(); t.bound = -1.f; }
+    SSD_HIP(hipStreamSynchronize(st));
+    std::vector<float> w, sc, sh;
+    for (const Layer& l : net->layers) {
+        if (l.kind != LK_CONV || l.kh != 1 || l.kw != 1 || l.head_kind != 0 || l.out < 0 || l.in < 0 || l.act != SSD_ACT_NONE || !l.packed) continue;
+        bool relu6_dw = false, other = false;
+        for (const Layer& d : net->layers) {
+            if (d.kind == LK_FUSED || d.out != l.in) continue;
+            if (d.kind == LK_DW && d.act == SSD_ACT_RELU6) relu6_dw = true; else other = true;
+        }
+        if (!relu6_dw || other) continue;
+        Tensor& to = net->tensors[l.out];
+        const Tensor* tr = l.res >= 0 ? &net->tensors[l.res] : nullptr;
+        if (tr && (tr->bound < 0.f || (int)tr->blo.size() != l.Cout)) continue;
+        const int kpad = conv_kpad(l.Cin);
+        w.resize((size_t)l.Cout * kpad);
+        SSD_HIP(hipMemcpy(w.data(), l.packed, w.size() * sizeof(float), hipMemcpyDeviceToHost));
+        sc.assign(l.Cout, 1.f);
+        sh.assign(l.Cout, 0.f);
+        if (l.scale) SSD_HIP(hipMemcpy(sc.data(), l.scale, l.Cout * sizeof(float), hipMemcpyDeviceToHost));
+        if (l.shift) SSD_HIP(hipMemcpy(sh.data(), l.shift, l.Cout * sizeof(float), hipMemcpyDeviceToHost));
+        std::vector<double> lo(l.Cout), hi(l.Cout);
+        const int ok = ssd_block_output_interval(w.data(), l.Cout, l.Cin, kpad, sc.data(), sh.data(), tr ? tr->blo.data() : nullptr,
+                                                 tr ? tr->bhi.data() : nullptr, lo.data(), hi.data());
+        if (ok < 0) return ok;
+        if (!ok) continue;
+        double m = 0.0;
+        for (int c = 0; c < l.Cout; ++c) m = std::max(m, std::max(std::fabs(lo[c]), std::fabs(hi[c])));
+        float b = (float)m;
+        if ((double)b < m) b = std::nextafter(b, INFINITY);
+        if (!std::isfinite(b)) continue;
+        to.blo = std::move(lo);
+        to.bhi = std::move(hi);
+        to.bound = b;
+    }
+    return SSD_OK;
+}
+
+static int finalize_image_f16x2(ssd_net* net, hipStream_t st) {
+    net->iplane_bytes = 0;
+    for (auto& f : net->layers) { f.fz_weh = f.fz_wph = nullptr; f.f16_ke = f.f16_kp = f.f16_s = 0; }
+    if (!net->image_f16x2 || net->precision != 0 || !net->image_split) return SSD_OK;
+    ScopedDev bits_dev;
+    SSD_HIP(hipMalloc((void**)&bits_dev.p, 2 * sizeof(unsigned)));
+    for (auto& f : net->layers) {
+        if (f.kind != LK_FUSED || f.f_type != 0 || f.in < 0 || !image_kernel_takes(*net, f)) continue;
+        int s = 0;
+        if (!ssd_f16x2_input_exp(net->tensors[f.in].bound, &s)) continue;
+        FusedBlockParams q = fused_shape(*net, f, 1);
+        q.bf16 = 2; q.groups = q.Ce / 32;
+        q.we3 = q.wp3 = reinterpret_cast<const short*>(f.fz_we);
+        if (!image_block2_supported(q)) continue;
+        const Layer& le = net->layers[f.f_expand];
+        const Layer& lp = net->layers[f.f_project];
+        unsigned bits[2] = {0, 0};
+        SSD_HIP(hipMemsetAsync(bits_dev.p, 0, 2 * sizeof(unsigned), st));
+        int rc = launch_absmax_bits(f.fz_we, le.Cin, le.Cout, reinterpret_cast<unsigned*>(bits_dev.p), st);
+        if (!rc) rc = launch_absmax_bits(f.fz_wp, lp.Cin, lp.Cout, reinterpret_cast<unsigned*>(bits_dev.p) + 1, st);
+        if (rc) return rc;
+        SSD_HIP(hipMemcpyAsync(bits, bits_dev.p, 2 * sizeof(unsigned), hipMemcpyDeviceToHost, st));
+        SSD_HIP(hipStreamSynchronize(st));
+        if (bits[0] >= 0x7f800000u || bits[1] >= 0x7f800000u) continue;
+        const int ke = conv_f16x2_weight_exp(bits[0]), kp = conv_f16x2_weight_exp(bits[1]);
+        if (std::abs(s + ke) > 100 || std::abs(8 + kp) > 100) continue;
+        f.f16_s = s; f.f16_ke = ke; f.f16_kp = kp;
+        const size_t fe = (conv_f16x2_plane_shorts(le.Cin, le.Cout) + 1) / 2, fp = (conv_f16x2_plane_shorts(lp.Cin, lp.Cout) + 1) / 2;
+        rc = dev_alloc(*net, fe, &f.fz_weh);
+        if (!rc) rc = dev_alloc(*net, fp, &f.fz_wph);
+        if (!rc) rc = launch_pack_f16x2(f.fz_we, le.Cin, le.Cout, f.f16_ke, reinterpret_cast<short*>(f.fz_weh), st, true);
+        if (!rc) rc = launch_pack_f16x2(f.fz_wp, lp.Cin, lp.Cout, f.f16_kp, reinterpret_cast<short*>(f.fz_wph), st, true);
+        if (rc) return rc;
+        net->iplane_bytes += (fe + fp) * sizeof(float);
+    }
+    return SSD_OK;
+}
+
 static int finalize_image_slabs(ssd_net* net, int max_batch, hipStream_t st) {
     size_t slab = 0;
     for (auto& f : net->layers) {
@@ -1242,6 +1363,8 @@
         if (rc) return rc;
     }
     rc = finalize_fused_weights(net, st);
+    if (!rc) rc = finalize_tensor_bounds(net, st);
+    if (!rc) rc = finalize_image_f16x2(net, st);
     if (!rc) rc = finalize_image_slabs(net, max_batch, st);
     if (!rc) rc = finalize_arena(net, max_batch, st);
     bool image_preset_ok = true;
@@ -1291,6 +1414,14 @@
         if (l.kind == LK_CONV && l.split_k > 1) sk += align_up((size_t)l.split_k * net->max_batch * l.Ho * l.Wo * l.Cout, 64);
     out[3] = sk * sizeof(float);
     return SSD_OK;
+}
+
+size_t ssd_net_image_f16x2_bytes(const ssd_net* net) { return net && net->finalized ? net->iplane_bytes : 0; }
+
+float ssd_net_tensor_bound(const ssd_net* net, const char* tensor) {
+    if (!net || !tensor || !net->finalized) return -1.f;
+    auto it = net->tensor_index.find(tensor);
+    return it == net->tensor_index.end() ? -1.f : net->tensors[it->second].bound;
 }
 
 int ssd_net_tuning_stats(const ssd_net* net, int* from_table, int* timed) {
@@ -1597,6 +1728,7 @@
     {"image_v2", &ssd_net::image_v2, nullptr, 0, 1, 0},
     {"conv_dma", &ssd_net::conv_dma, nullptr, 0, 1, 1},
     {"conv_f16x2", &ssd_net::conv_f16x2, nullptr, 0, 1, 1},
+    {"image_f16x2", &ssd_net::image_f16x2, nullptr, 0, 1, 1},
     {"plane_only", &ssd_net::plane_only, nullptr, 0, 1, 0},
     {"use_graph", &ssd_net::use_graph, nullptr, 0, 1, 0},
 };
@@ -1737,6 +1869,13 @@
     else snprintf(buf, sizeof(buf), "%s", conv_config_name(l.cfg));
     return buf;
 }
+int ssd_net_layer_image_form(const ssd_net* net, int i, int B) {
+    if (!net || i < 0 || i >= (int)net->layers.size() || B < 1) return -1;
+    const Layer& f = net->layers[i];
+    if (f.kind != LK_FUSED || (f.route != RT_IMAGE && f.route != RT_IMAGE_SPLIT)) return -1;
+    return fused_params(*net, f, B).bf16;
+}
+
 static double algorithmic_flops(const Layer& l, int B) {
     const double px = (double)B * l.Ho * l.Wo;
     if (l.kind == LK_CONV) return 2.0 * px * l.kh * l.kw * l.Cin * l.Cout;
diff --git a/tf-ssd_amd/models/_net.py b/tf-ssd_amd/models/_net.py
--- a/tf-ssd_amd/models/_net.py
+++ b/tf-ssd_amd/models/_net.py
@@ -8,7 +8,7 @@
 import ssd_hip as _h
 
 _TABLE_OPTIONS = ("use_wino", "image_split", "conv_dma")
-_REFINALIZE_OPTIONS = ("precision", "image_split", "use_wino", "conv_dma", "conv_f16x2")
+_REFINALIZE_OPTIONS = ("precision", "image_split", "use_wino", "conv_dma", "conv_f16x2", "image_f16x2")
 _STALE_WARNED = set()
 
 
@@ -301,7 +301,18 @@
     def memory_summary(self):
         out = (ctypes.c_size_t * 4)()
         _h.check(_h.lib().ssd_net_memory_bytes(self._net, out), "ssd_net_memory_bytes")
-        return {"arena": int(out[0]), "planes": int(out[1]), "image_slabs": int(out[2]), "splitk_slabs": int(out[3])}
+        return {"arena": int(out[0]), "planes": int(out[1]), "image_slabs": int(out[2]), "splitk_slabs": int(out[3]),
+                "image_weight_planes": int(_h.lib().ssd_net_image_f16x2_bytes(self._net))}
+
+    def tensor_bound(self, name):
+        b = float(_h.lib().ssd_net_tensor_bound(self._net, name.encode()))
+        return b if b >= 0 else None
+
+    def image_forms(self, B):
+        lib = _h.lib()
+        forms = {lib.ssd_net_layer_name(self._net, i).decode(): lib.ssd_net_layer_image_form(self._net, i, B)
+                 for i in range(lib.ssd_net_num_layers(self._net))}
+        return {k: v for k, v in forms.items() if v >= 0}
 
     def set_tuning(self, text):
         self._tuning_explicit = text
diff --git a/tf-ssd_amd/ssd_hip.py b/tf-ssd_amd/ssd_hip.py
--- a/tf-ssd_amd/ssd_hip.py
+++ b/tf-ssd_amd/ssd_hip.py
@@ -240,6 +240,13 @@
     "ssd_net_set_tuning": (ctypes.c_int, [vp, ctypes.c_char_p]),
     "ssd_net_tuning_stats": (ctypes.c_int, [vp, ctypes.POINTER(ctypes.c_int), ctypes.POINTER(ctypes.c_int)]),
     "ssd_net_memory_bytes": (ctypes.c_int, [vp, ctypes.POINTER(ctypes.c_size_t)]),
+    "ssd_net_image_f16x2_bytes": (ctypes.c_size_t, [vp]),
+    "ssd_net_tensor_bound": (ctypes.c_float, [vp, ctypes.c_char_p]),
+    "ssd_block_output_interval": (ctypes.c_int, [c_float_p, ctypes.c_int, ctypes.c_int, ctypes.c_int, c_float_p, c_float_p,
+                                                 ctypes.POINTER(ctypes.c_double), ctypes.POINTER(ctypes.c_double),
+                                                 ctypes.POINTER(ctypes.c_double), ctypes.POINTER(ctypes.c_double)]),
+    "ssd_f16x2_input_exp": (ctypes.c_int, [ctypes.c_float, c_int_p]),
+    "ssd_net_layer_image_form": (ctypes.c_int, [vp, ctypes.c_int, ctypes.c_int]),
     "ssd_build_id": (ctypes.c_char_p, []),
     "ssd_stream_create": (vp, [ctypes.c_int]),
     "ssd_stream_create_masked": (vp, [ctypes.POINTER(ctypes.c_uint), ctypes.c_int]),
```

Result: faster. 67810 (median of 6 runs) (+7.5%).
